# JJanai/slowflow

Hardware: AMD Instinct MI355X
Metric: Mpix*solver-iters/s at 1024x436 (whole coarse-to-fine path) (higher is better)
Workload: dtype f32

## Files before the change

### include/slowflow_amd.h

```cpp
#ifndef SLOWFLOW_AMD_H
#define SLOWFLOW_AMD_H

#include <stddef.h>

#ifdef __cplusplus
extern "C" {
#endif

#define SFA_VERSION 1
#define SFA_MAX_REF 8

typedef enum {
    SFA_OK = 0,
    SFA_ERR_ARG = -1,
    SFA_ERR_HIP = -2,
    SFA_ERR_NO_DEVICE = -3,
    SFA_ERR_REF_FRAME = -4,
    SFA_ERR_TIMEOUT = -5,
    SFA_ERR_UNSUPPORTED = -6
} sfa_status;

typedef struct sfa_image { int width, height, stride; float *data; } sfa_image;
typedef struct sfa_color_image { int width, height, stride; float *c1, *c2, *c3; } sfa_color_image;

// ... 263 lines not shown
int  sfa_job_download_alternation_occlusions(sfa_job *job, int b, int alter, float *occ, int stride);
double sfa_job_mpix_iters(const sfa_job *job);
double sfa_job_device_bytes(const sfa_job *job);

typedef enum { SFA_DEV_F32 = 0, SFA_DEV_U8 = 1, SFA_DEV_U16 = 2 } sfa_dev_dtype;
typedef struct sfa_dev_layout { int dtype; long long window, frame, channel, row, column; } sfa_dev_layout;
void sfa_dev_layout_default(sfa_dev_layout *l, int w, int h, int n_frames);
int  sfa_job_upload_device(sfa_job *job, int b0, int n, const void *frames_dev, const sfa_dev_layout *layout, const float *const chw[3]);
int  sfa_job_set_flow_device(sfa_job *job, int b0, int n, const float *flow_dev, const long long strides[4]);
int  sfa_job_download_device(sfa_job *job, int b0, int n, float *flow_dev, const long long strides[4], float *occ_dev, const long long occ_strides[3]);
int  sfa_job_changes(const sfa_job *job, int b0, int n, float *out);
int  sfa_sequence_upload_device(sfa_sequence *seq, int f0, int n, const void *frames_dev, const sfa_dev_layout *layout);
int  sfa_pair_job_upload_device(sfa_pair_job *job, int b0, int n, const void *frames_dev, const sfa_dev_layout *layout);
int  sfa_pair_job_set_flow_device(sfa_pair_job *job, int b0, int n, const float *flow_dev, const long long strides[4]);
int  sfa_pair_job_download_device(sfa_pair_job *job, int b0, int n, float *flow_dev, const long long strides[4]);
typedef struct sfa_mosaic_desc { int dtype; long long frame, row, column; int W, H, x0, y0; } sfa_mosaic_desc;
int  sfa_demosaic_device(sfa_ctx *ctx, int n, const void *mosaic_dev, const sfa_mosaic_desc *desc, int method, int red_x, int red_y, float *dst_dev,
                         const long long dst_strides[4], int w, int h);
int  sfa_sequence_upload_mosaic_device(sfa_sequence *seq, int f0, int n, const void *mosaic_dev, const sfa_mosaic_desc *desc, int method, int red_x, int red_y);
int  sfa_sequence_upload_mosaic(sfa_sequence *seq, int f, const void *mosaic_host, int dtype, long long host_stride, int W, int H, int x0, int y0, int method,
                                int red_x, int red_y);
int  sfa_job_set_raw_weights(sfa_job *job, int b0, int n, int red_x, int red_y, float weight);
int  sfa_sequence_rescale(sfa_sequence *dst_seq, int f_dst, sfa_sequence *src_seq, int f_src, int n, float scale);

int  sfa_ctx_wait_stream(sfa_ctx *ctx, void *stream);
int  sfa_ctx_signal_stream(sfa_ctx *ctx, void *stream);

typedef struct sfa_sor_batch sfa_sor_batch;
int  sfa_sor_batch_create(sfa_ctx *ctx, int w, int h, int batch, sfa_sor_batch **out);
void sfa_sor_batch_destroy(sfa_sor_batch *sb);
int  sfa_sor_batch_upload(sfa_sor_batch *sb, int b, const float *du, const float *dv, const float *a11, const float *a12,
                          const float *a22, const float *b1, const float *b2, const float *sh, const float *sv, int stride);
int  sfa_sor_batch_run(sfa_sor_batch *sb, int iterations, float omega);
int  sfa_sor_batch_download(sfa_sor_batch *sb, int b, float *du, float *dv, int stride);

int  sfa_ctx_set_wait_bound(sfa_ctx *ctx, unsigned spins);

int  sfa_debug_set(const char *name, const char *value);
int  sfa_ctx_set_verbose(sfa_ctx *ctx, int on);

int  sfa_pair_job_download_system(sfa_pair_job *job, int b, float *a11, float *a12, float *a22, float *b1, float *b2, int stride);

int  sfa_pyramid_down(sfa_ctx *ctx, float *dst, int dw, int dh, int dstride, const float *src, int sw, int sh, int sstride, int nplanes, int nb, float sigma,
                      int info[3]);
int  sfa_resize_flow(sfa_ctx *ctx, float *dwx, float *dwy, int dw, int dh, int dstride, const float *swx, const float *swy, int sw, int sh, int sstride, int nb,
                     float post_x, float post_y);
int  sfa_job_download_level_frame(sfa_job *job, int b, int level, int f, float *frame3, int stride);

int  sfa_division_chain(sfa_ctx *ctx, const float *numerators, const float *denominators, float *q_chain, float *q_exact, unsigned char *admitted, size_t n);

int  sfa_profile_enable(sfa_ctx *ctx, int on);
int  sfa_profile_read(sfa_ctx *ctx, int *n_sor_launches, double *sor_ms_total, double *sor_bytes_total);
int  sfa_profile_read_kernels(sfa_ctx *ctx, int *n_assembly_launches, double *assembly_ms_total, double *assembly_pixel_terms, char *sor_kernel, int sor_kernel_len);
int  sfa_timer_start(sfa_ctx *ctx);
int  sfa_timer_stop(sfa_ctx *ctx, float *ms);

#ifdef __cplusplus
}
#endif
#endif
```

### slowflow_amd/__init__.py

```python
import ctypes as C
import os
import subprocess
import weakref

import numpy as np

_HERE = os.path.dirname(os.path.abspath(__file__))
LIB_PATH = os.environ.get("SFA_LIB") or os.path.join(_HERE, "libslowflow_amd.so")
MAX_REF = 8
MOSAIC_TILE = (64, 16)
MOSAIC_DTYPES = {"float32": 0, "uint8": 1, "uint16": 2}

_f = C.POINTER(C.c_float)


class SlowflowError(RuntimeError):
    pass


def build(verbose=False):
    out = subprocess.run(["make", "-C", os.path.join(_HERE, "csrc"), "-j4"], capture_output=True, text=True)
    if out.returncode != 0:
        raise SlowflowError("building libslowflow_amd.so failed:\n" + out.stdout + out.stderr)
    if verbose:
# ... 122 lines not shown


def track_fill_params(**kw):
    f = TrackFillParams()
    lib().sfa_track_fill_params_default(C.byref(f))
    for k, v in kw.items():
        assert k in ("epic_skip", "min_size", "epic", "workspace_bytes"), k
        setattr(f, k, v)
    return f


def track_job_bytes(params, fill=None):
    L = lib()
    L.sfa_track_job_bytes.argtypes = [C.POINTER(TrackParams), C.POINTER(C.c_size_t)]
    L.sfa_track_job_bytes_fill.argtypes = [C.POINTER(TrackParams), C.POINTER(TrackFillParams), C.POINTER(C.c_size_t)]
    b = C.c_size_t()
    name = "sfa_track_job_bytes" if fill is None else "sfa_track_job_bytes_fill"
    rc = L.sfa_track_job_bytes(C.byref(params), C.byref(b)) if fill is None else L.sfa_track_job_bytes_fill(C.byref(params), C.byref(fill), C.byref(b))
    if rc != 0:
        raise SlowflowError("%s: %s" % (name, L.sfa_last_error(None).decode()))
    return b.value


EXPORTS = [
    "sfa_device_count", "sfa_ctx_create", "sfa_ctx_destroy", "sfa_last_error", "sfa_ctx_sync", "sfa_params_default",
    "sfa_variational", "sfa_variational_2frame", "sfa_variational_2frame_batch", "sfa_epic_nearest_seeds_batch", "sfa_epic_nn_stage_ms", "sfa_ctx_set_epic_search", "sfa_epic_nn_search_info", "sfa_epic_interpolate_batch", "sfa_epic_fit_stage_ms", "sfa_epic_batch", "sfa_epic_saliency_batch", "sfa_epic_batch_stage_ms", "sfa_params_2frame_default", "sfa_pair_job_create", "sfa_pair_job_destroy", "sfa_pair_job_upload", "sfa_pair_job_run", "sfa_pair_job_download", "sfa_pair_job_download_system", "sfa_flow_magnitude_quantile", "sfa_quantile_ranks", "sfa_flow_magnitude_quantiles_device", "sfa_accumulate_consistent", "sfa_accumulate_consistent_scaled", "sfa_jet_source_default", "sfa_jet_flow_resample", "sfa_jet_occlusion_decode", "sfa_hypothesis_energies_scaled", "sfa_accumulate_grid", "sfa_energy_params_default", "sfa_hypothesis_energies", "sfa_hypothesis_energies_ex", "sfa_dt_smoothness_weight", "sfa_fuse_params_default", "sfa_fuse_hypotheses", "sfa_consistent_regions", "sfa_fill_samples", "sfa_fill_matches", "sfa_fill_trajectories", "variational", "sfa_compute_one_level", "sfa_normalize", "sfa_sor_coupled", "sfa_sor_red_black", "sor_coupled",
    "sfa_image_warp", "sfa_derivative_stack", "sfa_convolve", "sfa_dpsis_weight", "sfa_smoothness", "sfa_sub_laplacian",
    "sfa_add_data_and_match", "sfa_occlusion_costs", "sfa_grid_cut", "sfa_grid_cut_batch", "sfa_gaussian_blur", "sfa_resize_linear", "sfa_resize_linear_fx", "sfa_gaussian_presmooth", "sfa_pyramid_sizes",
    "sfa_pyramid_down", "sfa_resize_flow", "sfa_job_download_level_frame",
    "sfa_sequence_create", "sfa_sequence_destroy", "sfa_sequence_upload", "sfa_sequence_download", "sfa_sequence_normalize", "sfa_sequence_frame_sums", "sfa_normalize_statistics", "sfa_sequence_apply_normalization",
    "sfa_job_create", "sfa_job_destroy", "sfa_job_upload", "sfa_job_upload_resident", "sfa_job_reset_flow", "sfa_job_run", "sfa_job_download", "sfa_job_download_occlusions", "sfa_job_keep_alternation_occlusions", "sfa_job_download_alternation_occlusions", "sfa_job_mpix_iters", "sfa_job_device_bytes",
    "sfa_dev_layout_default", "sfa_job_upload_device", "sfa_job_set_flow_device", "sfa_job_download_device", "sfa_job_changes", "sfa_pair_job_upload_device", "sfa_pair_job_set_flow_device", "sfa_pair_job_download_device", "sfa_sequence_upload_device", "sfa_ctx_wait_stream", "sfa_ctx_signal_stream",
    "sfa_demosaic_device", "sfa_sequence_upload_mosaic_device", "sfa_sequence_upload_mosaic", "sfa_job_set_raw_weights", "sfa_sequence_rescale",
    "sfa_sor_batch_create", "sfa_sor_batch_destroy", "sfa_sor_batch_upload", "sfa_sor_batch_run", "sfa_sor_batch_download",
    "sfa_track_params_default", "sfa_track_job_bytes", "sfa_track_job_create", "sfa_track_job_destroy", "sfa_track_job_upload_flows", "sfa_track_job_upload_frames", "sfa_track_job_upload_flows_device", "sfa_track_job_upload_frames_device", "sfa_track_job_run", "sfa_track_job_download_rate", "sfa_track_job_download_fused", "sfa_track_job_download_best", "sfa_ctx_free_bytes", "sfa_track_job_download_device", "sfa_track_job_stage_ms", "sfa_track_job_upload_occlusions_device", "sfa_track_job_download_rate_device", "sfa_track_job_download_best_device",
    "sfa_track_fill_params_default", "sfa_track_job_bytes_fill", "sfa_track_job_create_fill", "sfa_track_job_upload_fill", "sfa_track_job_upload_fill_device", "sfa_track_job_download_fill", "sfa_track_job_fill_ms", "sfa_track_job_fill_info",
    "sfa_division_chain", "sfa_ctx_set_wait_bound", "sfa_debug_set", "sfa_ctx_set_verbose", "sfa_profile_enable", "sfa_profile_read", "sfa_profile_read_kernels", "sfa_timer_start", "sfa_timer_stop",
]

_lib = None


def lib():
    global _lib
    if _lib is None:
        if not os.path.exists(LIB_PATH):
            raise SlowflowError(f"{LIB_PATH} is missing: build it with slowflow_amd.build() / make -C slowflow_amd/csrc "
                                "(there is no CPU fallback)")
        L = C.CDLL(LIB_PATH)
        L.sfa_last_error.restype = C.c_char_p
        L.sfa_last_error.argtypes = [C.c_void_p]
        L.sfa_job_mpix_iters.restype = C.c_double
        L.sfa_job_mpix_iters.argtypes = [C.c_void_p]
        L.sfa_job_device_bytes.restype = C.c_double
        L.sfa_job_device_bytes.argtypes = [C.c_void_p]
        for name in ("sfa_ctx_destroy", "sfa_job_destroy", "sfa_pair_job_destroy", "sfa_track_job_destroy", "sfa_sor_batch_destroy", "sfa_sequence_destroy"):
            if hasattr(L, name):
                getattr(L, name).restype = None
                getattr(L, name).argtypes = [C.c_void_p]
        _lib = L
    return _lib


def fptr(a):
    assert a.dtype == np.float32 and a.flags["C_CONTIGUOUS"], "fp32 C-contiguous planes only"
    return a.ctypes.data_as(_f)


def stride_of(w):
    return ((w + 3) // 4) * 4
# ... 1036 lines not shown

    def apply_normalization(self, avg, std, f0=0, n=None):
        a, s = (C.c_double * 3)(*avg), (C.c_double * 3)(*std)
        self.ctx._ck(lib().sfa_sequence_apply_normalization(self.h_, f0, self.n - f0 if n is None else n, a, s), "sfa_sequence_apply_normalization")

    def close(self):
        if self.h_:
            if self.ctx.h:
                lib().sfa_sequence_destroy(self.h_)
            self.h_ = C.c_void_p()

    def __del__(self):
        try:
            self.close()
        except Exception:
            pass


class SorBatch:

    def __init__(self, ctx, w, h, batch=1):
        self.ctx, self.w, self.h, self.batch = ctx, w, h, batch
        self.h_ = C.c_void_p()
        ctx._ck(lib().sfa_sor_batch_create(ctx.h, w, h, batch, C.byref(self.h_)), "sfa_sor_batch_create")
        ctx._children.add(self)

    def upload(self, b, du, dv, a11, a12, a22, b1, b2, sh, sv):
        stride = du.shape[1]
        self.ctx._ck(lib().sfa_sor_batch_upload(self.h_, b, *[fptr(a) for a in (du, dv, a11, a12, a22, b1, b2, sh, sv)], stride), "sfa_sor_batch_upload")

    def run(self, iterations, omega):
        self.ctx._ck(lib().sfa_sor_batch_run(self.h_, int(iterations), C.c_float(omega)), "sfa_sor_batch_run")

    def download(self, b):
        stride = stride_of(self.w)
        du, dv = np.zeros((self.h, stride), np.float32), np.zeros((self.h, stride), np.float32)
        self.ctx._ck(lib().sfa_sor_batch_download(self.h_, b, fptr(du), fptr(dv), stride), "sfa_sor_batch_download")
        return du, dv

    def close(self):
        if self.h_:
            if self.ctx.h:
                lib().sfa_sor_batch_destroy(self.h_)
            self.h_ = C.c_void_p()

    def __del__(self):
        try:
            self.close()
        except Exception:
            pass
```

### slowflow_amd/csrc/api.hip

```cpp
#include <algorithm>
#include <cmath>
#include <cstring>
#include <memory>
#include <mutex>

#include "sfa_internal.h"

#pragma clang fp contract(off)

namespace sfa {

thread_local std::string g_thread_err;

#ifndef SFA_RELEASE
Switches g_switches;
static const char *const kSwitchNames[Switches::N] = {
    "SFA_SOR_CHAIN", "SFA_SOR_BAND", "SFA_SOR_F", "SFA_SOR_CH", "SFA_SOR_LEAD", "SFA_CHAIN_LDS", "SFA_RB_TILE", "SFA_WARP_ALLJ", "SFA_NO_WARP_SMOOTH",
    "SFA_ASSEMBLE_GENERIC", "SFA_EXACT_DIV", "SFA_ASM_XCD", "SFA_NO_DIRECT_OPERANDS", "SFA_NO_UV_ALIAS", "SFA_DEBUG_ACTIVE", "SFA_UNFUSED", "SFA_SHARE_SOR",
    "SFA_PYRAMID_UNFUSED", "SFA_CUT_DISCHARGE", "SFA_CUT_INNER", "SFA_CUT_SUPER", "SFA_CUT_TAIL_INNER", "SFA_CUT_PER", "SFA_CUT_TAIL_PER", "SFA_CUT_TAIL_SUPER",
    "SFA_CUT_DEBUG", "SFA_CUT_NO_TAIL", "SFA_CUT_TAIL", "SFA_NO_EXACT_BREAK", "SFA_PAIR_UNFUSED", "SFA_EPIC_FIT_PLAIN", "SFA_EPIC_NN_SET", "SFA_EPIC_NN_SLICE"};
static int set_switch(const char *name, const char *value) {
    for (int i = 0; i < Switches::N; i++)
        if (!strcmp(name, kSwitchNames[i])) {
            g_switches.given[i] = value != nullptr;
            g_switches.value[i] = value ? atoi(value) : 0;
            if (i == Switches::EPIC_NN_SET && value) g_switches.value[i] = !strcmp(value, "sparse") ? 1 : !strcmp(value, "dense") ? 0 : -1;
            return SFA_OK;
        }
    return SFA_ERR_ARG;
}
static void switches_from_environment() {
    static std::once_flag once;
    std::call_once(once, [] {
        const char *d = getenv("SFA_DEBUG");
        if (!d || atoi(d) == 0) return;
        for (int i = 0; i < Switches::N; i++)
            if (const char *e = getenv(kSwitchNames[i])) (void)set_switch(kSwitchNames[i], e);
    });
}
#else
static void switches_from_environment() {}
#endif

int set_error(sfa_ctx *ctx, int code, const char *fmt, ...) {
    char buf[1024];
    va_list ap;
    va_start(ap, fmt);
    vsnprintf(buf, sizeof buf, fmt, ap);
    va_end(ap);
    g_thread_err = buf;
    if (ctx) ctx->err = buf;
    return code;
}
// ... 527 lines not shown
    long pl = 0, es = 0;
    DevMem mem;
    SorWorkspace ws;
    float *plane(int b, int i) const { return mem.f() + b * es + (long)i * pl; }
};

int sfa_sor_batch_create(sfa_ctx *ctx, int w, int h, int batch, sfa_sor_batch **out) {
    CHECK_ARGS(ctx && out && w > 0 && h > 0 && batch > 0 && batch <= kMaxBatch, "bad arguments");
    SFA_HIP(ctx, hipSetDevice(ctx->device));
    std::unique_ptr<sfa_sor_batch> sb(new sfa_sor_batch());
    sb->ctx = ctx; sb->w = w; sb->h = h; sb->nb = batch; sb->pitch = dev_pitch(w);
    sb->pl = (long)sb->pitch * h; sb->es = 9 * sb->pl;
    SFA_TRY(sb->mem.alloc(ctx, (size_t)batch * sb->es * sizeof(float)));
    SFA_HIP(ctx, hipMemsetAsync(sb->mem.p, 0, (size_t)batch * sb->es * sizeof(float), ctx->stream));
    *out = sb.release();
    return SFA_OK;
}
void sfa_sor_batch_destroy(sfa_sor_batch *sb) {
    if (!sb) return;
    (void)hipSetDevice(sb->ctx->device);
    (void)hipStreamSynchronize(sb->ctx->stream);
    delete sb;
}
int sfa_sor_batch_upload(sfa_sor_batch *sb, int b, const float *du, const float *dv, const float *a11, const float *a12, const float *a22, const float *b1,
                         const float *b2, const float *sh, const float *sv, int stride) {
    sfa_ctx *ctx = sb ? sb->ctx : nullptr;
    CHECK_ARGS(sb && b >= 0 && b < sb->nb && du && dv && a11 && a12 && a22 && b1 && b2 && sh && sv && stride >= sb->w, "bad arguments");
    SFA_HIP(ctx, hipSetDevice(ctx->device));
    const float *src[9] = {du, dv, a11, a12, a22, b1, b2, sh, sv};
    for (int i = 0; i < 9; i++) SFA_TRY(upload_plane(ctx, sb->plane(b, i), sb->pitch, src[i], stride, sb->w, sb->h));
    SFA_HIP(ctx, hipStreamSynchronize(ctx->stream));
    return SFA_OK;
}
int sfa_sor_batch_run(sfa_sor_batch *sb, int iterations, float omega) {
    sfa_ctx *ctx = sb ? sb->ctx : nullptr;
    CHECK_ARGS(sb, "null batch");
    SFA_HIP(ctx, hipSetDevice(ctx->device));
    Geo g{sb->w, sb->h, sb->pitch, sb->pl, sb->es, sb->nb, WMask::first(sb->nb), nullptr};
    return sor_run(ctx, sb->ws, g, sb->plane(0, 0), sb->plane(0, 1), sb->plane(0, 2), sb->plane(0, 3), sb->plane(0, 4), sb->plane(0, 5), sb->plane(0, 6),
                   sb->plane(0, 7), sb->plane(0, 8), iterations, omega, true);
}
int sfa_sor_batch_download(sfa_sor_batch *sb, int b, float *du, float *dv, int stride) {
    sfa_ctx *ctx = sb ? sb->ctx : nullptr;
    CHECK_ARGS(sb && b >= 0 && b < sb->nb && du && dv && stride >= sb->w, "bad arguments");
    SFA_HIP(ctx, hipSetDevice(ctx->device));
    SFA_TRY(download_plane(ctx, du, stride, sb->plane(b, 0), sb->pitch, sb->w, sb->h));
    SFA_TRY(download_plane(ctx, dv, stride, sb->plane(b, 1), sb->pitch, sb->w, sb->h));
    return sfa_ctx_sync(ctx);
}

int sfa_sor_coupled(sfa_ctx *ctx, sfa_image *du, sfa_image *dv, sfa_image *a11, sfa_image *a12, sfa_image *a22, sfa_image *b1, sfa_image *b2,
                    sfa_image *dpsis_horiz, sfa_image *dpsis_vert, int iterations, float omega) {
    CHECK_ARGS(ctx && du && dv && a11 && a12 && a22 && b1 && b2 && dpsis_horiz && dpsis_vert, "null image");
    const int w = du->width, h = du->height, stride = du->stride;
    CHECK_ARGS(w > 0 && h > 0 && stride >= w, "bad image geometry");
    sfa_image *im[9] = {du, dv, a11, a12, a22, b1, b2, dpsis_horiz, dpsis_vert};
    for (auto *i : im) CHECK_ARGS(i->data && i->width == w && i->height == h && i->stride == stride, "images must share one geometry");
    Staging s;
    SFA_TRY(s.init(ctx, w, h, 9));
    for (int i = 0; i < 9; i++) SFA_TRY(s.up(i, im[i]->data, stride));
    SorWorkspace ws;
    SFA_TRY(sor_run(ctx, ws, s.geo(), s.plane(0), s.plane(1), s.plane(2), s.plane(3), s.plane(4), s.plane(5), s.plane(6), s.plane(7), s.plane(8), iterations,
                    omega, true));
    SFA_TRY(s.down(du->data, stride, 0)); SFA_TRY(s.down(dv->data, stride, 1));
    if (!(w < 2 || h < 2 || iterations < 1))
        for (int i = 2; i < 5; i++) SFA_TRY(s.down(im[i]->data, stride, i));
// ... 378 lines not shown
```

### slowflow_amd/csrc/job.hip

```cpp
#include <algorithm>
#include <cmath>
#include <cstring>
#include <memory>
#include <vector>

#include "sfa_internal.h"

#pragma clang fp contract(off)

namespace sfa {

enum { P_WX = 0, P_WY, P_UU, P_VV, P_DU, P_DV, P_ODU, P_ODV, P_SH, P_SV, P_A11, P_A12, P_A22, P_B1, P_B2, P_OCC, P_DPSIS, P_COUNT };
struct Level {
    int w = 0, h = 0, pitch = 0, lstride = 0, ref = 0, F = 0, nb = 0;
    bool fused = true;
    long pl = 0, es = 0;
    long off_masks = 0, off_warp = 0, off_stacks = 0, off_tmp = 0;
    float *base = nullptr;
    float *pbase = nullptr;
    float *plane(int i) const { return i < 2 ? pbase + (long)i * pl : base + (long)(i - 2) * pl; }
    float *mask(int s) const { return base + off_masks + (long)s * pl; }
    float *stack(int s, int toref) const { return base + off_stacks + ((long)s * 2 + toref) * 24 * pl; }
    float *warp(int s, int sp1) const { return base + off_warp + (long)(s + sp1) * 3 * pl; }
    float *frame(int f) const { return pbase + 2 * pl + (long)f * 3 * pl; }
// ... 189 lines not shown
    SFA_HIP(c, hipStreamSynchronize(c->stream));
    for (int b = 0; b < L.nb; b++)
        if (close.test(b) && std::max(hx[2 * b], hx[2 * b + 1]) < p.thres_inner) in_active.clear(b);
    return SFA_OK;
}

static int inner_iterations(sfa_ctx *c, const Level &L, const sfa_params &p, const LevelPlan &P, AssembleArgs &aa, SorWorkspace &sorws, const Geo &g, bool smoothed) {
    if (!P.direct) launch_zero_planes(c, g, P.du, 2);
    WMask in_active = g.active, outer_done = WMask::none();
    for (int inner = 0; inner < p.niter_inner; inner++) {
        Geo gi = g;
        gi.active = in_active;
        const bool first_zero = P.direct && inner == 0;
        SFA_TRY(assemble_and_solve(c, L, p, P, aa, sorws, gi, first_zero, smoothed && inner == 0));
        if (update_flow(c, p, P, aa.op, gi, inner, first_zero)) outer_done = in_active;
        if (P.verbose) print_changes(c, L, "\tinner it", inner, in_active);
        if (P.thres_in && inner + 1 < p.niter_inner) {
            SFA_TRY(inner_break(c, L, p, P, gi, in_active));
            if (!in_active.any()) break;
        }
    }
    if (outer_done != g.active) {
        Geo go = g;
        go.active = g.active.andnot(outer_done);
        launch_update_outer(c, go, P.wx, P.wy, P.uu, P.vv, c->d_red, P.dfa, P.dfb);
    }
    return SFA_OK;
}
static int run_level(sfa_ctx *c, const Level &L, const sfa_params &p, const ChannelWeights &cw, SorWorkspace &sorws, DevMem &cut_scratch, float *change, float *occ_log) {
    AssembleArgs aa;
    bool need_toref[2 * SFA_MAX_REF] = {false};
    SFA_TRY(data_terms(c, L, p, cw, aa, need_toref));
    const LevelPlan P(c, L, p);
    const OuterBreak brk{c, P.thres_out};
    const WMask all = WMask::first(L.nb);
    Geo g = L.geo(all);
    launch_fill_planes(c, g, P.occ, 1, (p.one_direction || p.occlusion_reasoning) ? -1.0f : 0.0f);
    launch_dpsis(c, g, P.dpsis, L.frame(L.ref), L.es, 5.0f, p.norm_avg, p.norm_std, p.hbit);
    if (!P.uv_alias) launch_copy_planes(c, g, P.uu, P.wx, 2, L.es, L.es);
    g.amask = c->d_amask;
    SFA_HIP(c, hipMemsetAsync(c->d_last, 0, sizeof(LastBlock), c->stream));
    launch_set_mask(c, all);

    for (int alter = 0; alter < p.niter_alter; alter++) {
        WMask active = all;
        g.active = active;
        if (P.thres_out && alter > 0) launch_set_mask(c, all);
        bool smoothed = get_derivatives(c, L, p, g, need_toref, P.uv_alias);
        if (alter > 0 && p.occlusion_reasoning && !p.one_direction) SFA_TRY(optimize_occlusions(c, L, p, g, cut_scratch));
        if (alter > 0 && p.occlusion_reasoning && occ_log)
            launch_copy_planes(c, g, occ_log + (long)alter * L.pl, P.occ, 1, (long)p.niter_alter * L.pl, L.es);
        for (int outer = 0; outer < p.niter_outer; outer++) {
            SFA_TRY(brk.known(outer, active));
            if (!active.any()) break;
            if (sw_given(Switches::DEBUG_ACTIVE)) fprintf(stderr, "level %dx%d alter %d outer %d known active %d\n", L.w, L.h, alter, outer, active.count());
            g.active = active;
            if (outer > 0) smoothed = get_derivatives(c, L, p, g, need_toref, P.uv_alias);
            if (!L.fused) launch_mask_weight(c, g, L.mask(0), P.occ, aa.data_norm, L.ref, p.one_direction);
            SFA_TRY(inner_iterations(c, L, p, P, aa, sorws, g, smoothed));
            if (P.verbose) print_changes(c, L, "outer it", outer, active);
            const bool last_iter = (alter == p.niter_alter - 1 && outer == p.niter_outer - 1);
            if (P.thres_out || last_iter) launch_outer_threshold(c, g, c->d_red, P.thres_out ? p.thres_outer : 0.0f, P.dfa, P.dfb);
            SFA_TRY(brk.publish(outer));
        }
    }
    if (change) {
// ... 422 lines not shown
```

### slowflow_amd/csrc/kernels.hip

```cpp
#include "sfa_device.h"
#include "sor_device.h"

#pragma clang fp contract(off)

namespace sfa {

__device__ __forceinline__ float psi_vec(const PenaltyDev &p, float xsq) {
    const float e2 = p.eps * p.eps;
    switch (p.id) {
    case 0: return 1.0f;
    case 2: return __fdiv_rn(1.0f, 2.0f * e2 + xsq);
    case 3: {
        float out = __fdiv_rn(1.0f, 2.0f * sqrt_rn(xsq + e2));
        if (sqrt_rn(xsq) > p.trunc) out = 0.0f;
        return out;
    }
    case 4: {
        float t = e2 + xsq;
        t = t * t;
        return __fdiv_rn(e2 + 2.0f * xsq, t);
    }
    default: return __fdiv_rn(1.0f, 2.0f * sqrt_rn(xsq + e2));
    }
}
// ... 1304 lines not shown
            p.ixz[ch] = d5x_in(sZ[ch], cz);
        }
    }
    return p;
}
template <class K>
__device__ __forceinline__ void asm_epilogue_pixel(const AssembleArgs &a, const Geo &g, Acc &A, float u, float v, int x0, int y0, int tx, int yl, int x, int y) {
    const float *const lds = asm_lds<K>();
    const int gy0 = y0 + DT_H - 1;
    const TileAcc U{lds, x0, gy0}, V{lds + K::GR * DT_W, x0, gy0}, Hh{lds + 2 * K::GR * DT_W, x0, gy0}, Wv{lds + 3 * K::GR * DT_W, x0, gy0};
    if (a.do_laplacian) {
        A.b1 = laplacian_gather(A.b1, U, Hh, Wv, x, y, g.w, g.h);
        A.b2 = laplacian_gather(A.b2, V, Hh, Wv, x, y, g.w, g.h);
    }
    if (!a.op.sa) return;
    const float hp = Hh(x, y);
    const float hl = x > 0 ? Hh(x - 1, y) : 0.0f;
    const float vp = Wv(x, y);
    const float vt = y > 0 ? Wv(x, y - 1) : 0.0f;
    const PointBlock q = sor_point_block(hl, hp, vt, vp, y, g.h, A.a11, A.a12, A.a22);
    const OperandTile<K> T;
    T.A[yl][tx] = make_float4(q.i11, q.i12, q.i22, vt);
    T.B[yl][tx] = make_float4(A.b1, A.b2, hp, y < g.h - 1 ? vp : 0.0f);
    T.X[yl][tx] = make_float2(u, v);
}
template <class K>
__device__ __forceinline__ void asm_store_operand_tile(const SorOperandOut &op, const Geo &g, int b, int c0, int r0) {
    const OperandTile<K> T;
    for (int item = threadIdx.x; item < (DT_X + K::TY - 1) * K::TY; item += K::NT) {
        const int dl = item / K::TY, rl = item % K::TY, cl = dl - rl;
        if (cl < 0 || cl >= DT_X) continue;
        const int r = r0 + rl, c = c0 + cl;
        if (r >= g.h || c >= g.w) continue;
        const size_t e = diag_entry(b, op.ent, op.RP, op.G, c, r);
        if (SFA_X_AI & 64) continue;
        const float2 xv = T.X[rl][cl];
        op.sa[e] = T.A[rl][cl];
        op.sb[e] = T.B[rl][cl];
        op.x[e] = f2u(xv.x, xv.y);
    }
}

template <int TY, int NT, int MINB, bool ZUV, int FAST, bool XT>
__global__ void __launch_bounds__(NT, MINB) k_assemble_images(AssembleArgs a, const float *__restrict__ base, float *__restrict__ a11, float *__restrict__ a12,
                                                              float *__restrict__ a22, float *__restrict__ b1, float *__restrict__ b2,
                                                              const float *__restrict__ du, const float *__restrict__ dv, const float *__restrict__ uu,
                                                              const float *__restrict__ vv, const float *__restrict__ sh, const float *__restrict__ sv,
                                                              const float *__restrict__ occ, Geo g, XcdTiles xt) {
    using K = AsmTile<TY, NT>;
    constexpr int NR = K::NR, NP = K::NP;
    float *const lds = asm_lds<K>();
#ifdef SFA_ASM_TIMING
    unsigned long long at_acc[14] = {0}, at_t = __builtin_readcyclecounter();
#endif
    int bx, by, b;
    if (!asm_block_tile<XT>(g, xt, bx, by, b)) return;
    asm_reset_progress<K>(a.op, bx, by, b);
    if (!elem_active(g, b)) return;
    const int x0 = bx * DT_X - DT_H, y0 = by * TY - DT_H;
    const bool tile_in = SFA_TILE_FAST && x0 >= 0 && x0 + DT_W <= g.w && y0 >= 0 && y0 + K::TR <= g.h;
    const long eb = b * g.es;
    const int tx = threadIdx.x & 63;
    const int ty = __builtin_amdgcn_readfirstlane(threadIdx.x >> 6);
    const int x = x0 + DT_H + tx;
    const int dt_norm = FAST ? 1 : a.dt_norm;
    PenaltyDev pcolor = a.color, pgrad = a.grad;
    if (FAST) { pcolor.id = FAST; pgrad.id = FAST; }
// ... 165 lines not shown
    const int wid = threadIdx.y, lane = threadIdx.x;
    if (lane == 0) { sm[wid] = a; sm[BY + wid] = b; }
    __syncthreads();
    if (wid == 0 && lane == 0) {
        double sa = 0, sb = 0;
        for (int i = 0; i < BY; i++) { sa += sm[i]; sb += sm[BY + i]; }
        a = sa; b = sb;
    }
}

__global__ void __launch_bounds__(BX *BY) k_update_inner(float *__restrict__ uu, float *__restrict__ vv, const float *__restrict__ wx, const float *__restrict__ wy,
                                                          const float *__restrict__ du, const float *__restrict__ dv, const float *__restrict__ odu,
                                                          const float *__restrict__ odv, double *__restrict__ partial, float *__restrict__ dfa, float *__restrict__ dfb, Geo g) {
    const int b = blockIdx.z;
    const int x = blockIdx.x * BX + threadIdx.x;
    double sa = 0, sb = 0;
    if (elem_active(g, b) && x < g.w)
        for (int y = blockIdx.y * BY + threadIdx.y; y < g.h; y += gridDim.y * BY) {
            const size_t o = b * g.es + (size_t)y * g.pitch + x;
            const float d = du[o], e = dv[o];
            sa += (double)fabsf(odu[o] - d);
            sb += (double)fabsf(odv[o] - e);
            if (dfa) { dfa[o] = fabsf(odu[o] - d); dfb[o] = fabsf(odv[o] - e); }
            uu[o] = wx[o] + d;
            vv[o] = wy[o] + e;
        }
    block_sum2(sa, sb);
    if (threadIdx.x == 0 && threadIdx.y == 0) {
        const size_t blk = ((size_t)b * gridDim.y + blockIdx.y) * gridDim.x + blockIdx.x;
        partial[2 * blk] = sa; partial[2 * blk + 1] = sb;
    }
}
__global__ void __launch_bounds__(BX *BY) k_update_inner_x(float *__restrict__ uu, float *__restrict__ vv, const float *__restrict__ wx, const float *__restrict__ wy,
                                                            const unsigned long long *__restrict__ xs, long ent, int RP, int G, const float *__restrict__ odu,
                                                            const float *__restrict__ odv, float *__restrict__ du_out, float *__restrict__ dv_out,
                                                            double *__restrict__ partial, float *__restrict__ dfa, float *__restrict__ dfb, Geo g) {
    const int b = blockIdx.z;
    const int x = blockIdx.x * BX + threadIdx.x;
    double sa = 0, sb = 0;
    if (elem_active(g, b) && x < g.w)
        for (int y = blockIdx.y * BY + threadIdx.y; y < g.h; y += gridDim.y * BY) {
            const size_t o = b * g.es + (size_t)y * g.pitch + x;
            const unsigned long long xv = xs[diag_entry(b, ent, RP, G, x, y)];
            const float d = __uint_as_float((unsigned)(xv & 0xffffffffu)), e = __uint_as_float((unsigned)(xv >> 32));
            const float od = odu ? odu[o] : 0.0f, oe = odv ? odv[o] : 0.0f;
            sa += (double)fabsf(od - d);
            sb += (double)fabsf(oe - e);
            if (dfa) { dfa[o] = fabsf(od - d); dfb[o] = fabsf(oe - e); }
            uu[o] = wx[o] + d;
            vv[o] = wy[o] + e;
            if (du_out) { du_out[o] = d; dv_out[o] = e; }
        }
    block_sum2(sa, sb);
    if (threadIdx.x == 0 && threadIdx.y == 0) {
        const size_t blk = ((size_t)b * gridDim.y + blockIdx.y) * gridDim.x + blockIdx.x;
        partial[2 * blk] = sa; partial[2 * blk + 1] = sb;
    }
}
template <bool FUSE>
__global__ void __launch_bounds__(BX *BY) k_update_outer_x(float *__restrict__ uu, float *__restrict__ vv, float *__restrict__ wx, float *__restrict__ wy,
                                                            const unsigned long long *__restrict__ xs, long ent, int RP, int G, double *__restrict__ partial,
                                                            double *__restrict__ out, unsigned *__restrict__ done, float *__restrict__ dfa, float *__restrict__ dfb, Geo g) {
    __shared__ unsigned long long tX[16][67];
    const int b = blockIdx.z;
    const int tid = threadIdx.y * BX + threadIdx.x;
    const int c0 = blockIdx.x * 64;
    double sa = 0, sb = 0;
    if (!elem_active(g, b)) return;
    {
        for (int r0 = blockIdx.y * 16; r0 < g.h; r0 += gridDim.y * 16) {
            __syncthreads();
            for (int item = tid; item < (64 + 16 - 1) * 16; item += BX * BY) {
                const int dl = item / 16, rl = item % 16, cl = dl - rl;
                if (cl < 0 || cl >= 64) continue;
                const int r = r0 + rl, c = c0 + cl;
                if (r < g.h && c < g.w) tX[rl][cl] = xs[diag_entry(b, ent, RP, G, c, r)];
            }
            __syncthreads();
            const int x = c0 + threadIdx.x;
            if (x < g.w)
#pragma unroll
                for (int k = 0; k < 4; k++) {
                    const int rl = threadIdx.y + 4 * k, y = r0 + rl;
                    if (y >= g.h) break;
                    const size_t o = b * g.es + (size_t)y * g.pitch + x;
                    const unsigned long long xv = tX[rl][threadIdx.x];
                    const float d = __uint_as_float((unsigned)(xv & 0xffffffffu)), e = __uint_as_float((unsigned)(xv >> 32));
                    const float ox = wx[o], oy = wy[o];
                    const float u = ox + d, v = oy + e;
                    sa += (double)fabsf(u - ox);
                    sb += (double)fabsf(v - oy);
                    if (uu) { uu[o] = u; vv[o] = v; }
                    if (dfa) { dfa[o] = fabsf(u - ox); dfb[o] = fabsf(v - oy); }
#if defined(SFA_UPD_NT) && SFA_UPD_NT
                    __builtin_nontemporal_store(u, wx + o); __builtin_nontemporal_store(v, wy + o);
#else
                    wx[o] = u; wy[o] = v;
#endif
                }
        }
    }
    block_sum2(sa, sb);
    if (!FUSE) {
        if (tid == 0) {
            const size_t blk = ((size_t)b * gridDim.y + blockIdx.y) * gridDim.x + blockIdx.x;
            partial[2 * blk] = sa; partial[2 * blk + 1] = sb;
        }
        return;
    }
// ... 123 lines not shown
    if (!which.test(b)) return;
    float fa, fd;
    exact_norms(dfa + b * g.es, dfb + b * g.es, g, lane, fa, fd);
    if (lane == 0) { out[2 * b] = fa; out[2 * b + 1] = fd; }
}
void launch_exact_norms(sfa_ctx *c, const Geo &g, const float *dfa, const float *dfb, const WMask &which, float *out) {
    hipLaunchKernelGGL(k_exact_norms, dim3(g.nb), dim3(64), 0, c->stream, dfa, dfb, out, which, g);
}
__global__ void k_set_mask(unsigned long long *amask, WMask v) { for (int i = 0; i < kMaskWords; i++) amask[i] = v.w[i]; }
static unsigned long long *unsure_of(sfa_ctx *c) { return c->d_last->unsure; }
void launch_outer_threshold(sfa_ctx *c, const Geo &g, const double *red, float thres, const float *dfa, const float *dfb) {
    const bool exact = dfa && thres > 0.0f;
    hipLaunchKernelGGL(k_outer_threshold, dim3(kMaskWords), dim3(64), 0, c->stream, red, c->d_last->last, c->d_amask, g.active, g.nb, (double)g.h * g.w, thres,
                       exact ? unsure_of(c) : (unsigned long long *)nullptr, break_band(g.w, g.h));
    if (exact) hipLaunchKernelGGL(k_exact_break, dim3(g.nb), dim3(64), 0, c->stream, dfa, dfb, c->d_last->last, c->d_amask, unsure_of(c), g, thres);
}
void launch_set_mask(sfa_ctx *c, const WMask &v) { hipLaunchKernelGGL(k_set_mask, dim3(1), dim3(1), 0, c->stream, c->d_amask, v); }

static double *partials_of(sfa_ctx *c) { return c->d_red + 2 * kMaxBatch; }
constexpr int kRedRows = 16;
static inline dim3 red_grid(const Geo &g, int z) { return dim3((g.w + BX - 1) / BX, std::min((g.h + BY - 1) / BY, kRedRows), z); }

void launch_update_inner(sfa_ctx *c, const Geo &g, float *uu, float *vv, const float *wx, const float *wy, const float *du, const float *dv,
                         const float *old_du, const float *old_dv, double *red, float *dfa, float *dfb) {
    dim3 grid = red_grid(g, g.nb);
    const int per_elem = grid.x * grid.y;
    hipLaunchKernelGGL(k_update_inner, grid, block2d(), 0, c->stream, uu, vv, wx, wy, du, dv, old_du, old_dv, partials_of(c), dfa, dfb, g);
    hipLaunchKernelGGL(k_reduce_partials, dim3(g.nb), dim3(256), 0, c->stream, partials_of(c), per_elem, red, g.active, g.amask);
}
void launch_update_inner_x(sfa_ctx *c, const Geo &g, float *uu, float *vv, const float *wx, const float *wy, const SorOperandOut &x, const float *old_du,
                           const float *old_dv, float *du_out, float *dv_out, double *red, float *dfa, float *dfb) {
    dim3 grid = red_grid(g, g.nb);
    const int per_elem = grid.x * grid.y;
    hipLaunchKernelGGL(k_update_inner_x, grid, block2d(), 0, c->stream, uu, vv, wx, wy, x.x, x.ent, x.RP, x.G, old_du, old_dv, du_out, dv_out, partials_of(c), dfa, dfb, g);
    hipLaunchKernelGGL(k_reduce_partials, dim3(g.nb), dim3(256), 0, c->stream, partials_of(c), per_elem, red, g.active, g.amask);
}
constexpr int kFuseReduceWindows = 4;
void launch_update_outer_x(sfa_ctx *c, const Geo &g, float *uu, float *vv, float *wx, float *wy, const SorOperandOut &x, double *red, float *dfa, float *dfb) {
    dim3 grid((g.w + 63) / 64, std::min((g.h + 15) / 16, kRedRows), g.nb);
    const int per_elem = grid.x * grid.y;
    unsigned *done = c->d_last->done;
    if (g.nb <= kFuseReduceWindows) {
        hipLaunchKernelGGL(k_update_outer_x<true>, grid, block2d(), 0, c->stream, uu, vv, wx, wy, x.x, x.ent, x.RP, x.G, partials_of(c), red, done, dfa, dfb, g);
        return;
    }
    hipLaunchKernelGGL(k_update_outer_x<false>, grid, block2d(), 0, c->stream, uu, vv, wx, wy, x.x, x.ent, x.RP, x.G, partials_of(c), red, done, dfa, dfb, g);
    hipLaunchKernelGGL(k_reduce_partials, dim3(g.nb), dim3(256), 0, c->stream, partials_of(c), per_elem, red, g.active, g.amask);
}
void launch_update_outer(sfa_ctx *c, const Geo &g, float *wx, float *wy, const float *uu, const float *vv, double *red, float *dfa, float *dfb) {
    dim3 grid = red_grid(g, g.nb);
    const int per_elem = grid.x * grid.y;
    hipLaunchKernelGGL(k_update_outer, grid, block2d(), 0, c->stream, wx, wy, uu, vv, partials_of(c), dfa, dfb, g);
    hipLaunchKernelGGL(k_reduce_partials, dim3(g.nb), dim3(256), 0, c->stream, partials_of(c), per_elem, red, g.active, g.amask);
}

__global__ void k_copy_planes(float *__restrict__ dst, const float *__restrict__ src, Geo g, int nplanes, long dst_es, long src_es) {
    const int b = blockIdx.z / nplanes, pl = blockIdx.z % nplanes;
    if (!elem_active(g, b)) return;
    const int x = blockIdx.x * BX + threadIdx.x, y = blockIdx.y * BY + threadIdx.y;
    if (x >= g.w || y >= g.h) return;
    const size_t o = pl * g.pl + (size_t)y * g.pitch + x;
    dst[b * dst_es + o] = src[b * src_es + o];
}
void launch_copy_planes(sfa_ctx *c, const Geo &g, float *dst, const float *src, int nplanes, long dst_es, long src_es) {
    hipLaunchKernelGGL(k_copy_planes, grid2d(g, nplanes), block2d(), 0, c->stream, dst, src, g, nplanes, dst_es, src_es);
}

__global__ void k_fill_planes(float *__restrict__ p, Geo g, int nplanes, float v) {
    const int b = blockIdx.z / nplanes, pl = blockIdx.z % nplanes;
    if (!elem_active(g, b)) return;
    const int x = blockIdx.x * BX + threadIdx.x, y = blockIdx.y * BY + threadIdx.y;
    if (x >= g.pitch || y >= g.h) return;
    p[b * g.es + pl * g.pl + (size_t)y * g.pitch + x] = v;
}
void launch_fill_planes(sfa_ctx *c, const Geo &g, float *p, int nplanes, float v) {
    dim3 grid((g.pitch + BX - 1) / BX, (g.h + BY - 1) / BY, g.nb * nplanes);
    hipLaunchKernelGGL(k_fill_planes, grid, block2d(), 0, c->stream, p, g, nplanes, v);
}
void launch_zero_planes(sfa_ctx *c, const Geo &g, float *p, int nplanes) { launch_fill_planes(c, g, p, nplanes, 0.0f); }
// ... 436 lines not shown
```

### slowflow_amd/csrc/sfa_internal.h

```cpp
#pragma once
#include <hip/hip_runtime.h>

#include <cstdarg>
#include <cstdio>
#include <string>
#include <vector>

#include "../../include/slowflow_amd.h"
#include "dev_view.h"

#pragma clang fp contract(off)

namespace sfa {

constexpr int kMaskWords = 2;
constexpr int kMaxBatch = 64 * kMaskWords;
struct WMask {
    unsigned long long w[kMaskWords];
    __host__ __device__ bool test(int b) const { return (w[b >> 6] >> (b & 63)) & 1ull; }
    __host__ __device__ void clear(int b) { w[b >> 6] &= ~(1ull << (b & 63)); }
    __host__ __device__ void set(int b) { w[b >> 6] |= 1ull << (b & 63); }
    __host__ __device__ bool any() const { unsigned long long o = 0; for (int i = 0; i < kMaskWords; i++) o |= w[i]; return o != 0; }
    __host__ __device__ bool operator==(const WMask &o) const { bool e = true; for (int i = 0; i < kMaskWords; i++) e = e && w[i] == o.w[i]; return e; }
    __host__ __device__ bool operator!=(const WMask &o) const { return !(*this == o); }
// ... 43 lines not shown
    size_t ev_used = 0;
    double sor_bytes = 0;
    std::vector<hipEvent_t> ev2;
    size_t ev2_used = 0;
    double asm_pixel_terms = 0;
    char sor_kernel[160] = {0};
    void *rb_tmp = nullptr;
    size_t rb_tmp_bytes = 0;
    void *q_tmp = nullptr;
    size_t q_tmp_bytes = 0;
    float epic_ms[5] = {};
    int epic_search = 0;
    long long epic_info[4] = {};
    float epic_fit_ms[2] = {};
    float epic_batch_ms[8] = {};
    int epic_chain_runs[2] = {};
    hipEvent_t t0 = nullptr, t1 = nullptr;
    hipEvent_t ev_wait = nullptr, ev_signal = nullptr;
    bool verbose_changes = false;
    int cu_count = 256;
};

namespace sfa {

constexpr int kRedDoubles = 1 << 20;

int set_error(sfa_ctx *ctx, int code, const char *fmt, ...);
extern thread_local std::string g_thread_err;

struct Switches {
    enum Id {
        SOR_CHAIN, SOR_BAND, SOR_F, SOR_CH, SOR_LEAD, CHAIN_LDS, RB_TILE, WARP_ALLJ, NO_WARP_SMOOTH, ASSEMBLE_GENERIC, EXACT_DIV, ASM_XCD, NO_DIRECT_OPERANDS,
        NO_UV_ALIAS, DEBUG_ACTIVE, UNFUSED, SHARE_SOR, PYRAMID_UNFUSED, CUT_DISCHARGE, CUT_INNER, CUT_SUPER, CUT_TAIL_INNER, CUT_PER, CUT_TAIL_PER, CUT_TAIL_SUPER,
        CUT_DEBUG, CUT_NO_TAIL, CUT_TAIL, NO_EXACT_BREAK, PAIR_UNFUSED, EPIC_FIT_PLAIN, EPIC_NN_SET, EPIC_NN_SLICE, N
    };
    bool given[N] = {};
    int value[N] = {};
};
#ifdef SFA_RELEASE
#define SFA_FULL(...)
#else
#define SFA_FULL(...) __VA_ARGS__
#endif
#ifdef SFA_RELEASE
constexpr bool sw_given(Switches::Id) { return false; }
constexpr int sw_int(Switches::Id, int dflt) { return dflt; }
#else
extern Switches g_switches;
inline bool sw_given(Switches::Id i) { return g_switches.given[i]; }
inline int sw_int(Switches::Id i, int dflt) { return g_switches.given[i] ? g_switches.value[i] : dflt; }
#endif

#define SFA_HIP(ctx, call)                                                                         \
    do {                                                                                           \
        hipError_t _e = (call);                                                                    \
        if (_e != hipSuccess)                                                                      \
            return sfa::set_error((ctx), SFA_ERR_HIP, "%s failed: %s (%s:%d)", #call, hipGetErrorString(_e), __FILE__, __LINE__); \
    } while (0)

#define SFA_TRY(expr)            \
    do {                         \
        int _rc = (expr);        \
        if (_rc != SFA_OK) return _rc; \
    } while (0)

#define CHECK_ARGS_FN(fn, cond, msg) do { if (!(cond)) return sfa::set_error(ctx, SFA_ERR_ARG, "%s: %s", fn, msg); } while (0)
#define CHECK_ARGS(cond, msg) CHECK_ARGS_FN(__func__, cond, msg)
// ... 93 lines not shown
struct EpicChainDev { const float *const *cost; const float *const *matches; const int *nm; const float *const *sal; float *const *fx; float *const *fy; };
int epic_chain_device(sfa_ctx *ctx, const char *fn, int n, int w, int h, const sfa_epic_params *p, const EpicChainDev &io, int *rc, int (*counts)[3],
                      size_t workspace_bytes, int *status);

struct Geo { int w, h, pitch; long pl; long es; int nb; WMask active; const unsigned long long *amask; };

struct PenaltyDev { int id; float eps, trunc; };
inline PenaltyDev pen(const sfa_penalty &p) { return PenaltyDev{p.id, p.eps, p.trunc}; }

struct WarpJob { long src_off, dst_off, mask_off; int factor; };
struct WarpJobs { WarpJob job[4 * SFA_MAX_REF]; int n; };
void launch_warp_jobs(sfa_ctx *c, const Geo &g, const WarpJobs &J, float *base, const float *wx, const float *wy);
bool launch_warp_smooth(sfa_ctx *c, const Geo &g, const WarpJobs &J, float *base, const float *wx, const float *wy, int method, float *sh, float *sv,
                        const float *dpsis, float alpha, PenaltyDev reg);
void launch_warp(sfa_ctx *c, const Geo &g, float *dst3, float *mask, const float *src3, const float *wx, const float *wy, int factor,
                 long src_es );
void launch_deriv_stack(sfa_ctx *c, const Geo &g, float *out24, const float *I1, const float *I2, long es1, long es2);
void launch_convolve(sfa_ctx *c, const Geo &g, float *dst, const float *src, int order, int horiz, int nplanes);
void launch_dpsis(sfa_ctx *c, const Geo &g, float *dst, const float *im3, long im_es, float coef, const float avg[3], const float stdv[3], int hbit);
void launch_smoothness(sfa_ctx *c, const Geo &g, int method, float *sh, float *sv, const float *uu, const float *vv, const float *dpsis,
                       float alpha, PenaltyDev reg);
void launch_sub_laplacian(sfa_ctx *c, const Geo &g, float *dst, const float *src, const float *wh, const float *wv);
void launch_mask_weight(sfa_ctx *c, const Geo &g, float *masks, const float *occ, float data_norm, int ref, int one_direction);
void launch_fill(sfa_ctx *c, float *p, size_t n, float v);
void launch_division_chain(sfa_ctx *c, const float *a, const float *b, float *q_chain, float *q_exact, unsigned char *admitted, size_t n);
void launch_fill_planes(sfa_ctx *c, const Geo &g, float *p, int nplanes, float v);
void launch_zero_planes(sfa_ctx *c, const Geo &g, float *p, int nplanes);
void launch_outer_threshold(sfa_ctx *c, const Geo &g, const double *red, float thres, const float *dfa = nullptr, const float *dfb = nullptr);
void launch_set_mask(sfa_ctx *c, const WMask &v);

struct SorOperandOut {
    float4 *sa = nullptr, *sb = nullptr; unsigned long long *x = nullptr; unsigned *flags = nullptr;
    long ent = 0; int RP = 0, G = 0, ntasks = 0, nb = 0;
};
struct Term {
    long stack_off; long mask_off; float hd, hg, s; int is_ref;
    long i1_off, i2_off; int backward;
};
struct AssembleArgs {
    Term t[kMaxTerms];
    int n;
    int dt_norm;
    PenaltyDev color, grad;
    const float *chw; long chw_pl; long chw_es; int chw_pitch; int chw_stride0; int lstride;
    int accumulate;
    int do_laplacian;
    float data_norm; int one_direction;
    SorOperandOut op;
    int zero_duv;
    int chain_ok = 0;
};
void launch_assemble(sfa_ctx *c, const Geo &g, const AssembleArgs &a, const float *base , float *a11, float *a12,
                     float *a22, float *b1, float *b2, const float *du, const float *dv, const float *uu, const float *vv, const float *sh, const float *sv);

int launch_assemble_images(sfa_ctx *c, const Geo &g, const AssembleArgs &a, const float *base, float *a11, float *a12, float *a22, float *b1, float *b2,
                            const float *du, const float *dv, const float *uu, const float *vv, const float *sh, const float *sv, const float *occ);

void launch_smoothness_2f(sfa_ctx *c, const Geo &g, float *sh, float *sv, const float *uu, const float *vv, const float *dpsis, float half_alpha);
void launch_data_2f(sfa_ctx *c, const Geo &g, const float *D, const float *mask, const float *du, const float *dv, float *a11, float *a12, float *a22, float *b1,
                    float *b2, const float *wx, const float *wy, const float *sh, const float *sv, float hd, float hg);
void launch_data_2f_fused(sfa_ctx *c, const Geo &g, const float *I1, const float *I2, const float *mask, const float *du, const float *dv, float *a11, float *a12,
                          float *a22, float *b1, float *b2, const float *wx, const float *wy, const float *sh, const float *sv, float hd, float hg);

struct OccSlot {
    long s1_off, s2_off;
    long r1_off, r2_off;
// ... 25 lines not shown
                        long ses, int nb, float post_x, float post_y);
void launch_resize_scaled(sfa_ctx *c, float *dst, int dw, int dh, int dpitch, long dpl, long des, const float *src, int sw, int sh, int spitch, long spl,
                          long ses, int nplanes, int nb, float post_scale, double scale_x, double scale_y);
struct PyrInfo { int fused, td, lds; };
bool launch_pyr_down(sfa_ctx *c, float *dst, int dw, int dh, int dpitch, long dpl, long des, const float *src, int sw, int sh, int spitch, long spl, long ses,
                     int nplanes, int nb, const float *taps, int radius, PyrInfo *info = nullptr);
int pyramid_step(sfa_ctx *c, float *dst, int dw, int dh, int dpitch, long dpl, long des, const float *src, int sw, int sh, int spitch, long spl, long ses, int nplanes,
                 int nb, const float *taps, int radius, float *tmp, PyrInfo *info = nullptr);
void launch_presmooth(sfa_ctx *c, const Geo &g, float *dst, float *tmp, const float *src, int nplanes, float sigma);
void launch_normalize_sums(sfa_ctx *c, const Geo &g, const float *frames3, double *red );
void launch_normalize_apply(sfa_ctx *c, const Geo &g, float *frames3, const double avg[3], const double stdv[3]);
__attribute__((visibility("hidden"))) int cv_gauss_taps(float sigma, float k[kMaxBlurTaps]);

struct PackSrc { const void *p; int dtype; long long sw, sf, sc, sr, sx; };
void launch_pack_frames(sfa_ctx *c, float *dst, long dst_es, long pl, int pitch, int w, int h, int nwin, int F, const PackSrc &s);
void launch_pack_flow(sfa_ctx *c, float *dst, long dst_es, long pl, int pitch, int w, int h, int nwin, const float *src, const long long st[4]);
void launch_unpack_planes(sfa_ctx *c, const float *wx, const float *wy, const float *occ, long src_es, int pitch, int w, int h, int nwin, float *flow,
                          const long long st[4], float *occ_dst, const long long ost[3]);

struct MosaicSrc { const void *p; int dtype; long long sf, sr, sx; int W, H, x0, y0; };
struct MosaicDst { float *p; long long sf, sc, sr, sx; int w, h; };
void launch_demosaic(sfa_ctx *c, const MosaicSrc &src, const MosaicDst &dst, int n, int method, int red_x, int red_y);
void launch_raw_weights(sfa_ctx *c, float *chw, long es, long pl, int cp, int stride, int w, int h, int nwin, int red_x, int red_y, float weight);

struct SorWorkspace {
    sfa_ctx *ctx = nullptr;
    int w = 0, h = 0, K = 0, nb = 0;
    int NB = 0, NG = 0, RP = 0, ND = 0, G = 0, NS = 0, NCH = 0, ntasks = 0, F = 0, CHK = 0;
    int nwords = 0;
    long ent = 0;
    int band = 0, Wp = 0, EP = 0;
    int chain = 0;
    long edge_job = 0;
    DevMem sa, sb, x, flags, order, edge;
    int configure(sfa_ctx *ctx, int w, int h, int K, int nb);
};
int sor_operand_target(sfa_ctx *c, SorWorkspace &ws, const Geo &g, int K, SorOperandOut *out);
int sor_run_prepared(sfa_ctx *c, SorWorkspace &ws, const Geo &g, float *du, float *dv, int K, float omega);
int sor_rb_run(sfa_ctx *c, const Geo &g, float *du, float *dv, float *a11, float *a12, float *a22, const float *b1, const float *b2, const float *sh,
               const float *sv, int K, float omega);
int sor_run(sfa_ctx *c, SorWorkspace &ws, const Geo &g, float *du, float *dv, float *a11, float *a12, float *a22, const float *b1, const float *b2,
            const float *sh, const float *sv, int K, float omega, bool inv_out);

__attribute__((visibility("hidden"))) int check_view(sfa_ctx *ctx, const char *fn, const View &v, long long min_inner = 1);
__attribute__((visibility("hidden"))) int check_disjoint(sfa_ctx *ctx, const char *fn, std::initializer_list<View> views, const char *why = nullptr);
int check_frames_source(sfa_ctx *ctx, const char *fn, const void *frames_dev, const sfa_dev_layout *l, long long win_stride, int nwin, int F, int w, int h);
int check_device_pointer(sfa_ctx *ctx, const char *fn, const char *arg, const void *p, long long last, size_t elem);
int check_download_destination(sfa_ctx *ctx, const char *fn, int n, int w, int h, float *flow_dev, const long long strides[4], float *occ_dev,
                               const long long occ_strides[3]);
int check_batch_range(sfa_ctx *ctx, const char *fn, const char *what, int b0, int n, int nb);
__attribute__((visibility("hidden"))) int check_mosaic_method(sfa_ctx *ctx, const char *fn, int method, int red_x, int red_y);

}

struct sfa_pair_job {
    enum { WX, WY, UU, VV, DU, DV, SH, SV, A11, A12, A22, B1, B2, MASK, DPS, IM1, IM2 = IM1 + 3, WIM2 = IM2 + 3, NPL = WIM2 + 3 };
    sfa_ctx *ctx = nullptr;
    int w = 0, h = 0, n = 0, pitch = 0;
    long pl = 0, es = 0;
    sfa_params_2frame p;
    bool stored_stack = false;
    sfa::DevMem mem;
    sfa::DevMem stack;
    sfa::SorWorkspace ws;
    float *plane(int b, int i) const { return mem.f() + b * es + (long)i * pl; }
    sfa::Geo geo() const { return sfa::Geo{w, h, pitch, pl, es, n, sfa::WMask::first(n), nullptr}; }
// ... 17 lines not shown
```

### slowflow_amd/csrc/sor.hip

```cpp
#include <type_traits>

#include "sfa_internal.h"
#include "sfa_device.h"
#include "sor_device.h"

#pragma clang fp contract(off)

namespace sfa {

#ifndef SFA_BAND_STARTLAG
#define SFA_BAND_STARTLAG 2
#endif
#ifndef SFA_PUBLISH_VMCNT
#define SFA_PUBLISH_VMCNT (2 * CH - 1)
#endif

#ifndef SFA_PROGRESS_STRIDE
#define SFA_PROGRESS_STRIDE 32
#endif
constexpr int kProgressStride = SFA_PROGRESS_STRIDE;

struct SorArgs {
    const float4 *sa;
    const float4 *sb;
// ... 494 lines not shown
    constexpr int WINA = 2 * (FA - 1) * (64 + FA - 1) * 32, WINB_ = FB > 1 ? 2 * (FB - 1) * (64 + FB - 1) * 32 : 0;
    unsigned char *win0 = smem + (size_t)(NW - 1) * RING * 64 * 8 + 256;
    unsigned long long(*est0)[MC] = reinterpret_cast<unsigned long long(*)[MC]>(win0 + (size_t)NA * WINA + (size_t)NB_ * WINB_);
    constexpr int TVB = (FA + 1) * CH;
    unsigned long long *tvb0 = reinterpret_cast<unsigned long long *>(est0 + (size_t)NW * FA);
    unsigned &s_ticket = lprog[NW];
    const int lane = threadIdx.x & 63;
    const int wave = __builtin_amdgcn_readfirstlane(threadIdx.x >> 6);
    if (threadIdx.x == 0) s_ticket = atomicAdd(a.gflags + (size_t)a.nb * a.NB * NW * kProgressStride, 1u);
    if (threadIdx.x < NW) lprog[threadIdx.x] = 0;
    __syncthreads();
    const unsigned t = __builtin_amdgcn_readfirstlane(s_ticket);
    if (t >= (unsigned)(a.nb * a.NB)) return;
    const int job = t % a.nb, b = t / a.nb;
    if (!elem_active(a.active, a.amask, job)) return;
    unsigned char *win = wave < NA ? win0 + (size_t)wave * WINA : win0 + (size_t)NA * WINA + (size_t)(wave - NA) * WINB_;
    unsigned long long(*est)[MC] = est0 + (size_t)wave * FA;
    unsigned long long *tvb = tvb0 + (size_t)wave * TVB;
    const int k0 = wave < NA ? wave * FA : NA * FA + (wave - NA) * FB;
    if (wave == 0)                   band_wave<FA, CH, MC, RING, 0, FA>(a, ring, lprog, win, est, tvb, job, b, wave, lane, k0);
    else if (wave < NA)              band_wave<FA, CH, MC, RING, 1, FA>(a, ring, lprog, win, est, tvb, job, b, wave, lane, k0);
    else if (wave == NA && NB_ == 1) band_wave<FB, CH, MC, RING, 2, FA>(a, ring, lprog, win, est, tvb, job, b, wave, lane, k0);
    else if (wave == NA)             band_wave<FB, CH, MC, RING, 1, FA>(a, ring, lprog, win, est, tvb, job, b, wave, lane, k0);
    else if (wave == NW - 1)         band_wave<FB, CH, MC, RING, 2, FB>(a, ring, lprog, win, est, tvb, job, b, wave, lane, k0);
    else                             band_wave<FB, CH, MC, RING, 1, FB>(a, ring, lprog, win, est, tvb, job, b, wave, lane, k0);
}

struct PrepArgs {
    float4 *sa; float4 *sb; unsigned long long *x; unsigned *flags;
    const float *du, *dv, *b1, *b2, *sh, *sv;
    float *a11, *a12, *a22;
    long ent, es;
    int W, H, RP, ND, G, pitch, ntasks, nb, inv_out;
    WMask active; const unsigned long long *amask;
};
constexpr int PT_C = 64, PT_R = 16;
__global__ void __launch_bounds__(256) k_sor_prepare(PrepArgs p) {
    __shared__ float4 tA[PT_R][PT_C + 2];
    __shared__ float4 tB[PT_R][PT_C + 2];
    __shared__ float2 tX[PT_R][PT_C + 3];
    const int job = blockIdx.z;
    const int c0 = blockIdx.x * PT_C, r0 = blockIdx.y * PT_R;
    const int tx = threadIdx.x & 63, ty = threadIdx.x >> 6;
    if (blockIdx.x == 0 && blockIdx.y == 0) {
        for (int i = threadIdx.x; i < p.ntasks; i += 256) p.flags[(size_t)job * p.ntasks + i] = 0;
        if (job == 0 && threadIdx.x == 0) p.flags[(size_t)p.nb * p.ntasks] = 0;
    }
    if (!elem_active(p.active, p.amask, job)) return;
#pragma unroll
    for (int i = 0; i < PT_R / 4; i++) {
        const int rl = ty + 4 * i, r = r0 + rl, c = c0 + tx;
        if (r < p.H && c < p.W) {
            const size_t o = (size_t)job * p.es + (size_t)r * p.pitch + c;
            const float hp = p.sh[o];
            const float hl = c > 0 ? p.sh[o - 1] : 0.0f;
            const float vp = p.sv[o];
            const float vt = r > 0 ? p.sv[o - p.pitch] : 0.0f;
            const PointBlock q = sor_point_block(hl, hp, vt, vp, r, p.H, p.a11[o], p.a12[o], p.a22[o]);
            tA[rl][tx] = make_float4(q.i11, q.i12, q.i22, vt);
            tB[rl][tx] = make_float4(p.b1[o], p.b2[o], hp, r < p.H - 1 ? vp : 0.0f);
            tX[rl][tx] = make_float2(p.du[o], p.dv[o]);
            if (p.inv_out) { p.a11[o] = q.i11; p.a12[o] = q.i12; p.a22[o] = q.i22; }
        }
    }
    __syncthreads();
    for (int item = threadIdx.x; item < (PT_C + PT_R - 1) * PT_R; item += 256) {
        const int dl = item / PT_R, rl = item % PT_R, cl = dl - rl;
        if (cl < 0 || cl >= PT_C) continue;
        const int r = r0 + rl, c = c0 + cl;
        if (r >= p.H || c >= p.W) continue;
        const size_t e = diag_entry(job, p.ent, p.RP, p.G, c, r);
        p.sa[e] = tA[rl][cl];
        p.sb[e] = tB[rl][cl];
        const float2 xv = tX[rl][cl];
        p.x[e] = f2u(xv.x, xv.y);
    }
}

__global__ void k_sor_finish(float *__restrict__ du, float *__restrict__ dv, const unsigned long long *__restrict__ x, long ent, long es, int W, int H,
                             int RP, int G, int pitch, WMask active, const unsigned long long *__restrict__ amask) {
    const int job = blockIdx.z;
    const int c = blockIdx.x * 64 + threadIdx.x, r = blockIdx.y * 4 + threadIdx.y;
    if (c >= W || r >= H || !elem_active(active, amask, job)) return;
    const float2 v = u2f(x[diag_entry(job, ent, RP, G, c, r)]);
    const size_t o = (size_t)job * es + (size_t)r * pitch + c;
    du[o] = v.x;
    dv[o] = v.y;
}

__global__ void k_sor_readable(float *du_, float *dv_, const float *a11_, const float *a12_, const float *a22_, const float *b1_, const float *b2_,
                               const float *sh_, const float *sv_, long es, int w, int h, int stride, int iterations, float omega,
                               WMask active, const unsigned long long *amask) {
    if (threadIdx.x != 0 || !elem_active(active, amask, blockIdx.x)) return;
    const long eb = (long)blockIdx.x * es;
    float *du = du_ + eb, *dv = dv_ + eb;
    const float *a11 = a11_ + eb, *a12 = a12_ + eb, *a22 = a22_ + eb, *b1 = b1_ + eb, *b2 = b2_ + eb, *sh = sh_ + eb, *sv = sv_ + eb;
    for (int iter = 0; iter < iterations; iter++)
        for (int j = 0; j < h; j++)
            for (int i = 0; i < w; i++) {
                const size_t o = (size_t)j * stride + i;
                float sigma_u = 0.0f, sigma_v = 0.0f, sum_dpsis = 0.0f;
                if (j > 0) { sigma_u -= sv[o - stride] * du[o - stride]; sigma_v -= sv[o - stride] * dv[o - stride]; sum_dpsis += sv[o - stride]; }
                if (i > 0) { sigma_u -= sh[o - 1] * du[o - 1]; sigma_v -= sh[o - 1] * dv[o - 1]; sum_dpsis += sh[o - 1]; }
                if (j < h - 1) { sigma_u -= sv[o] * du[o + stride]; sigma_v -= sv[o] * dv[o + stride]; sum_dpsis += sv[o]; }
                if (i < w - 1) { sigma_u -= sh[o] * du[o + 1]; sigma_v -= sh[o] * dv[o + 1]; sum_dpsis += sh[o]; }
                const float A11 = a11[o] + sum_dpsis, A12 = a12[o], A22 = a22[o] + sum_dpsis;
                const float det = A11 * A22 - A12 * A12;
                const float B1 = b1[o] - sigma_u, B2 = b2[o] - sigma_v;
                du[o] = (1.0f - omega) * du[o] + __fdiv_rn(omega * (A22 * B1 - A12 * B2), det);
                dv[o] = (1.0f - omega) * dv[o] + __fdiv_rn(omega * (-A12 * B1 + A11 * B2), det);
            }
}

__global__ void __launch_bounds__(256) k_rb_invert(float *__restrict__ a11, float *__restrict__ a12, float *__restrict__ a22, const float *__restrict__ sh,
                                                   const float *__restrict__ sv, Geo g) {
    const int b = blockIdx.z;
    if (!elem_active(g, b)) return;
// ... 124 lines not shown
        float *tu = static_cast<float *>(c->rb_tmp), *tv = tu + (size_t)g.nb * pl;
        const dim3 grid((g.w + 63) / 64, (g.h + 15) / 16, g.nb);
        bool in_tmp = false;
        for (int k = 0; k < K; k += T) {
            const int ns = std::min(T, K - k);
            const float *iu = in_tmp ? tu : du, *iv = in_tmp ? tv : dv;
            float *ou = in_tmp ? du : tu, *ov = in_tmp ? dv : tv;
            const long ei = in_tmp ? pl : g.es, eo = in_tmp ? g.es : pl;
#ifndef SFA_RELEASE
            if (T == 3) hipLaunchKernelGGL((k_rb_tile<3>), grid, dim3(256), 0, c->stream, iu, iv, ei, g.pitch, ou, ov, eo, g.pitch, a11, a12, a22, b1, b2, sh, sv, g, ns, omega);
            else
#endif
                        hipLaunchKernelGGL((k_rb_tile<5>), grid, dim3(256), 0, c->stream, iu, iv, ei, g.pitch, ou, ov, eo, g.pitch, a11, a12, a22, b1, b2, sh, sv, g, ns, omega);
            in_tmp = !in_tmp;
        }
        if (in_tmp) {
            Geo gc = g;
            launch_copy_planes(c, gc, du, tu, 1, g.es, pl);
            launch_copy_planes(c, gc, dv, tv, 1, g.es, pl);
        }
    }
    if (prof) {
        (void)hipEventRecord(c->ev[c->ev_used + 1], c->stream);
        c->ev_used += 2;
        c->sor_bytes += (44.0 * K + 12.0) * (double)g.w * g.h * g.nb;
    }
    SFA_HIP(c, hipGetLastError());
    return SFA_OK;
}

bool chain_shape(int id, int K, int *KG, int *NW, int *FMAX);
int chain_ch();
int chain_shift(int id);
void chain_kernel_name(int id, int NG, char *buf, size_t n);
int chain_flag_stride();
int chain_ah();
int sor_chain_launch(sfa_ctx *c, SorWorkspace &ws, const Geo &g, int K, float omega);

static int chain_choice(int K, int nb, int NBands) {
    int id = 0;
    if (sw_given(Switches::SOR_CHAIN)) id = sw_int(Switches::SOR_CHAIN, 0);
    else if (sw_given(Switches::SOR_BAND) || sw_given(Switches::SOR_F)) id = 0;
    else {
        const int bands = nb * NBands;
        static const int lone[] = {16, 6, 1, 2, 5, 3, 0}, few[] = {6, 1, 2, 5, 3, 0}, many[] = {14, 11, 3, 5, 2, 6, 1, 0};
        int KG, NW, FMAX;
        for (const int *cand = bands <= 32 ? lone : bands <= 72 ? few : many; *cand; cand++)
            if (chain_shape(*cand, K, &KG, &NW, &FMAX)) { id = *cand; break; }
    }
    int KG, NW, FMAX;
    if (id > 0 && !chain_shape(id, K, &KG, &NW, &FMAX)) id = 0;
    return id;
}
static int band_shape(int K, int nb) {
#ifdef SFA_RELEASE
    (void)K; (void)nb;
    return 0;
#endif
    int F = nb >= 8 ? 43 : 0;
    F = sw_int(Switches::SOR_BAND, F);
    if (F == 43) { if (K == 30) return 43; F = 5; }
    if (F <= 0 || F > 6 || F == 4) return 0;
    auto fits = [&](int f) { return f >= 1 && K % f == 0 && K / f <= (f == 6 ? 5 : f == 5 ? 6 : f == 3 ? 10 : 16); };
    if (fits(F)) return F;
    if (fits(5)) return 5;
    if (fits(3)) return 3;
// ... 2 lines not shown
    return 0;
}
#ifndef SFA_BAND_CH3
#define SFA_BAND_CH3 4
#endif
#ifndef SFA_BAND_CH2
#define SFA_BAND_CH2 2
#endif
#ifndef SFA_BAND_CH5
#define SFA_BAND_CH5 4
#endif
constexpr int band_ch(int F) { return F == 3 ? SFA_BAND_CH3 : F == 5 ? SFA_BAND_CH5 : F == 6 ? 5 : F == 2 ? SFA_BAND_CH2 : 2; }
#ifndef SFA_BAND_MC3
#define SFA_BAND_MC3 12
#endif
#ifndef SFA_BAND_MC2
#define SFA_BAND_MC2 8
#endif
#ifndef SFA_BAND_MC5
#define SFA_BAND_MC5 8
#endif
constexpr int band_mc(int F) { return F == 3 ? SFA_BAND_MC3 : F == 2 ? SFA_BAND_MC2 : F == 5 ? SFA_BAND_MC5 : F == 6 ? 10 : 8; }
static int band_ring(int F) { return F == 2 ? 8 : 16; }
static size_t band_window(int F) { return F > 1 ? (size_t)2 * (F - 1) * (64 + F - 1) * 32 : 0; }

static void sor_shape(int K, int nwaves1, int &F, int &CHK) {
    F = nwaves1 >= 900 ? 2 : 1; CHK = F == 1 ? 16 : 8;
    F = sw_int(Switches::SOR_F, F);
    CHK = sw_int(Switches::SOR_CH, CHK);
    if (!((F == 1 && (CHK == 8 || CHK == 16)) || (F == 2 && (CHK == 8 || CHK == 4)) || (F == 3 && CHK == 4))) { F = 2; CHK = 8; }
    if (K % F != 0) { F = 1; CHK = 16; }
}

int SorWorkspace::configure(sfa_ctx *c, int w_, int h_, int K_, int nb_) {
    int F_, CH_;
    const int chain_ = chain_choice(K_, nb_, (h_ + K_ - 1 + 63) / 64);
    const int band_ = chain_ ? 0 : band_shape(K_, nb_);
    if (chain_) { F_ = 0; CH_ = chain_ch(); }
    else if (band_ == 43) { F_ = 4; CH_ = 12; }
    else if (band_) { F_ = band_; CH_ = band_mc(band_); }
    else sor_shape(K_, nb_ * ((h_ + K_ - 1 + 63) / 64) * K_, F_, CH_);
    if (ctx == c && w == w_ && h == h_ && K == K_ && nb == nb_ && F == F_ && CHK == CH_ && band == band_ && chain == chain_) return SFA_OK;
    ctx = c; w = w_; h = h_; K = K_; nb = nb_; F = F_; CHK = CH_; band = band_; chain = chain_;
    NB = (h + K - 1 + 63) / 64;
    if (chain) {
        int KG, NW, FMAX;
        chain_shape(chain, K, &KG, &NW, &FMAX);
        const int CH = chain_ch(), AH = chain_ah(), LEAD = AH + 1;
        NG = K / KG;
#ifndef SFA_GUARD_ALIGN
#define SFA_GUARD_ALIGN 8
#endif
        G = round_up(K + 64, SFA_GUARD_ALIGN);
        RP = round_up(h + 2 * G, 16);
        NCH = round_up((w + 64 + KG - NW + 2 * CH + FMAX + CH - 1) / CH + chain_shift(chain), 4);
        NS = round_up(NCH + LEAD + NW + 2, AH);
        ND = NS * CH + 64 * NB + G + 32;
        ntasks = NB * NG;
        nwords = ntasks * chain_flag_stride();
        ent = (long)ND * RP;
        EP = 256;
        Wp = round_up(EP + NS * CH + 64 + 2 * K + 64, 8);
        edge_job = (long)NB * K * Wp;
        SFA_TRY(edge.alloc(c, (size_t)nb * edge_job * sizeof(unsigned long long)));
        SFA_HIP(c, hipMemsetAsync(edge.p, 0, (size_t)nb * edge_job * sizeof(unsigned long long), c->stream));
        SFA_TRY(sa.alloc(c, (size_t)nb * ent * sizeof(float4)));
        SFA_TRY(sb.alloc(c, (size_t)nb * ent * sizeof(float4)));
        SFA_TRY(x.alloc(c, (size_t)nb * ent * sizeof(unsigned long long)));
        SFA_TRY(flags.alloc(c, ((size_t)nb * nwords + 16) * sizeof(unsigned)));
        SFA_TRY(order.alloc(c, (size_t)NB * NG * sizeof(int2)));
        SFA_HIP(c, hipMemsetAsync(sa.p, 0, (size_t)nb * ent * sizeof(float4), c->stream));
        SFA_HIP(c, hipMemsetAsync(sb.p, 0, (size_t)nb * ent * sizeof(float4), c->stream));
        SFA_HIP(c, hipMemsetAsync(x.p, 0, (size_t)nb * ent * sizeof(unsigned long long), c->stream));
        std::vector<int2> ord;
        ord.reserve(NB * NG);
        for (int key = 0; key <= 3 * (NB - 1) + (NG - 1); key++)
            for (int b = 0; b < NB; b++) {
                const int g = key - 3 * b;
                if (g >= 0 && g < NG) ord.push_back(make_int2(b, g));
            }
        SFA_HIP(c, hipMemcpyAsync(order.p, ord.data(), ord.size() * sizeof(int2), hipMemcpyHostToDevice, c->stream));
        SFA_HIP(c, hipStreamSynchronize(c->stream));
        return SFA_OK;
    }
    NG = band == 43 ? 8 : (K + F - 1) / F;
    G = K + 64;
    RP = round_up(h + 2 * G, 16);
    NS = w + 63 + F - 1;
    NCH = (NS + CHK - 1) / CHK;
    if (band) NS = NCH * CHK;
    ND = w + 64 * NB + 2 * CHK + F + 2 * G + 8;
    ntasks = NB * NG;
    nwords = ntasks * kProgressStride;
    ent = (long)ND * RP;
    if (band) {
        EP = 72;
        Wp = round_up(EP + NS + 2 * CHK + 8, 8);
        edge_job = (long)NB * K * Wp;
        SFA_TRY(edge.alloc(c, (size_t)nb * edge_job * sizeof(unsigned long long)));
        SFA_HIP(c, hipMemsetAsync(edge.p, 0, (size_t)nb * edge_job * sizeof(unsigned long long), c->stream));
    }
    SFA_TRY(sa.alloc(c, (size_t)nb * ent * sizeof(float4)));
    SFA_TRY(sb.alloc(c, (size_t)nb * ent * sizeof(float4)));
    SFA_TRY(x.alloc(c, (size_t)nb * ent * sizeof(unsigned long long)));
    SFA_TRY(flags.alloc(c, ((size_t)nb * nwords + 16) * sizeof(unsigned)));
    SFA_TRY(order.alloc(c, (size_t)ntasks * sizeof(int2)));
    SFA_HIP(c, hipMemsetAsync(sa.p, 0, (size_t)nb * ent * sizeof(float4), c->stream));
    SFA_HIP(c, hipMemsetAsync(sb.p, 0, (size_t)nb * ent * sizeof(float4), c->stream));
    SFA_HIP(c, hipMemsetAsync(x.p, 0, (size_t)nb * ent * sizeof(unsigned long long), c->stream));
    std::vector<int2> ord;
    ord.reserve(ntasks);
    for (int key = 0; key <= 3 * (NB - 1) + (NG - 1); key++)
        for (int b = 0; b < NB; b++) {
            const int g = key - 3 * b;
            if (g >= 0 && g < NG) ord.push_back(make_int2(b, g));
        }
    SFA_HIP(c, hipMemcpyAsync(order.p, ord.data(), ord.size() * sizeof(int2), hipMemcpyHostToDevice, c->stream));
    SFA_HIP(c, hipStreamSynchronize(c->stream));
    return SFA_OK;
}

int sor_operand_target(sfa_ctx *c, SorWorkspace &ws, const Geo &g, int K, SorOperandOut *out) {
    if (g.w < 2 || g.h < 2 || K < 1) return set_error(c, SFA_ERR_ARG, "sor_operand_target: system too small for the pipelined solver");
    SFA_TRY(ws.configure(c, g.w, g.h, K, g.nb));
    out->sa = (float4 *)ws.sa.p; out->sb = (float4 *)ws.sb.p; out->x = (unsigned long long *)ws.x.p; out->flags = (unsigned *)ws.flags.p;
    out->ent = ws.ent; out->RP = ws.RP; out->G = ws.G; out->ntasks = ws.nwords; out->nb = g.nb;
    return SFA_OK;
}

static int sor_launch_solve(sfa_ctx *c, SorWorkspace &ws, const Geo &g, float *du, float *dv, int K, float omega);

int sor_run(sfa_ctx *c, SorWorkspace &ws, const Geo &g, float *du, float *dv, float *a11, float *a12, float *a22, const float *b1, const float *b2,
            const float *sh, const float *sv, int K, float omega, bool inv_out) {
    if (g.w < 2 || g.h < 2 || K < 1) {
        hipLaunchKernelGGL(k_sor_readable, dim3(g.nb), dim3(64), 0, c->stream, du, dv, a11, a12, a22, b1, b2, sh, sv, g.es, g.w, g.h, g.pitch, K, omega,
                           g.active, g.amask);
        return SFA_OK;
    }
    SFA_TRY(ws.configure(c, g.w, g.h, K, g.nb));
    PrepArgs p;
    p.sa = (float4 *)ws.sa.p; p.sb = (float4 *)ws.sb.p; p.x = (unsigned long long *)ws.x.p; p.flags = (unsigned *)ws.flags.p;
    p.du = du; p.dv = dv; p.b1 = b1; p.b2 = b2; p.sh = sh; p.sv = sv; p.a11 = a11; p.a12 = a12; p.a22 = a22;
    p.ent = ws.ent; p.es = g.es; p.W = g.w; p.H = g.h; p.RP = ws.RP; p.ND = ws.ND; p.G = ws.G; p.pitch = g.pitch;
    p.ntasks = ws.nwords; p.nb = g.nb; p.inv_out = inv_out ? 1 : 0; p.active = g.active; p.amask = g.amask;
    hipLaunchKernelGGL(k_sor_prepare, dim3((g.w + PT_C - 1) / PT_C, (g.h + PT_R - 1) / PT_R, g.nb), dim3(256), 0, c->stream, p);
    return sor_launch_solve(c, ws, g, du, dv, K, omega);
}

int sor_run_prepared(sfa_ctx *c, SorWorkspace &ws, const Geo &g, float *du, float *dv, int K, float omega) {
    if (ws.ctx != c || ws.w != g.w || ws.h != g.h || ws.K != K || ws.nb != g.nb) return set_error(c, SFA_ERR_ARG, "sor_run_prepared: workspace not configured for this system");
    return sor_launch_solve(c, ws, g, du, dv, K, omega);
}

static int sor_launch_solve(sfa_ctx *c, SorWorkspace &ws, const Geo &g, float *du, float *dv, int K, float omega) {
    struct { float4 *sa, *sb; unsigned long long *x; unsigned *flags; } p{(float4 *)ws.sa.p, (float4 *)ws.sb.p, (unsigned long long *)ws.x.p, (unsigned *)ws.flags.p};
    SorArgs a;
    a.sa = p.sa; a.sb = p.sb; a.x = p.x; a.flags = p.flags; a.order = (const int2 *)ws.order.p; a.err = c->d_err;
    a.ent = ws.ent; a.W = g.w; a.H = g.h; a.K = K; a.NB = ws.NB; a.NG = ws.NG; a.RP = ws.RP; a.G = ws.G; a.NS = ws.NS; a.NCH = ws.NCH;
    a.ntasks = ws.ntasks; a.nwords = ws.nwords; a.nb = g.nb; a.omega = omega; a.active = g.active; a.amask = g.amask;
    const bool prof = c->profile && c->ev_used + 2 <= c->ev.size();
    if (prof) (void)hipEventRecord(c->ev[c->ev_used], c->stream);
    if (ws.chain) chain_kernel_name(ws.chain, ws.NG, c->sor_kernel, sizeof c->sor_kernel);
    else if (ws.band == 43) snprintf(c->sor_kernel, sizeof c->sor_kernel, "k_sor_band_mixed<4,6,3,2,4,12,16>");
    else if (ws.band) snprintf(c->sor_kernel, sizeof c->sor_kernel, "k_sor_band<%d>", ws.F);
    else snprintf(c->sor_kernel, sizeof c->sor_kernel, "k_sor_solve<%d,%d>", ws.F, ws.CHK);
    if (ws.chain) {
        SFA_TRY(sor_chain_launch(c, ws, g, K, omega));
    }
#ifndef SFA_RELEASE
    else if (ws.band) {
        BandArgs ba;
        ba.sa = p.sa; ba.sb = p.sb; ba.x = p.x; ba.edge = (unsigned long long *)ws.edge.p; ba.gflags = p.flags; ba.err = c->d_err;
        ba.ent = ws.ent; ba.edge_job = ws.edge_job; ba.W = g.w; ba.H = g.h; ba.K = K; ba.NB = ws.NB; ba.NW = ws.NG; ba.RP = ws.RP; ba.G = ws.G;
        ba.lead = band_ring(ws.F);
        if (sw_given(Switches::SOR_LEAD)) ba.lead = std::max(band_ch(ws.F) + 2, std::min(sw_int(Switches::SOR_LEAD, 0), band_ring(ws.F)));
        ba.NS = ws.NS; ba.NCH = ws.NCH; ba.nb = g.nb; ba.Wp = ws.Wp; ba.EP = ws.EP; ba.omega = omega; ba.active = g.active; ba.amask = g.amask;
        const dim3 bgrid(g.nb * ws.NB), bblock(ws.NG * 64);
        const size_t tvb = (ws.F + 1) * band_ch(ws.F) <= 64 ? (size_t)(ws.F + 1) * band_ch(ws.F) * 8 : 0;
        const size_t lds = (size_t)(ws.NG - 1) * band_ring(ws.F) * 64 * 8 + 256 + ws.NG * band_window(ws.F) + (size_t)ws.NG * ws.F * band_mc(ws.F) * 8 + ws.NG * tvb;
        if (ws.band == 43) {
            const size_t lds43 = (size_t)7 * 16 * 64 * 8 + 256 + 6 * (size_t)(2 * 3 * 67 * 32) + 2 * (size_t)(2 * 2 * 66 * 32) + (size_t)8 * 4 * 12 * 8 + (size_t)8 * 5 * 4 * 8;
            hipLaunchKernelGGL((k_sor_band_mixed<4, 6, 3, 2, 4, 12, 16>), bgrid, bblock, lds43, c->stream, ba);
        } else if (ws.F == 6) hipLaunchKernelGGL((k_sor_band<6, 5, band_ch(6), band_mc(6), 16>), bgrid, bblock, lds, c->stream, ba);
        else if (ws.F == 5) hipLaunchKernelGGL((k_sor_band<5, 6, band_ch(5), band_mc(5), 16>), bgrid, bblock, lds, c->stream, ba);
        else if (ws.F == 3) hipLaunchKernelGGL((k_sor_band<3, 10, band_ch(3), band_mc(3), 16>), bgrid, bblock, lds, c->stream, ba);
        else if (ws.F == 2) hipLaunchKernelGGL((k_sor_band<2, 16, band_ch(2), band_mc(2), 8>), bgrid, bblock, lds, c->stream, ba);
        else                hipLaunchKernelGGL((k_sor_band<1, 16, band_ch(1), band_mc(1), 16>), bgrid, bblock, lds, c->stream, ba);
    }
#endif
    else {
    const dim3 sgrid(g.nb * ws.ntasks), sblock(64);
    if (ws.F == 1 && ws.CHK == 16)      hipLaunchKernelGGL((k_sor_solve<1, 16>), sgrid, sblock, 0, c->stream, a);
    SFA_FULL(else if (ws.F == 1)                 hipLaunchKernelGGL((k_sor_solve<1, 8>), sgrid, sblock, 0, c->stream, a);)
    else if (ws.F == 2 && ws.CHK == 8)  hipLaunchKernelGGL((k_sor_solve<2, 8>), sgrid, sblock, 0, c->stream, a);
    SFA_FULL(else if (ws.F == 2)                 hipLaunchKernelGGL((k_sor_solve<2, 4>), sgrid, sblock, 0, c->stream, a);)
    SFA_FULL(else if (ws.F == 3)                 hipLaunchKernelGGL((k_sor_solve<3, 4>), sgrid, sblock, 0, c->stream, a);)
    else return set_error(c, SFA_ERR_ARG, "sor_launch_solve: no task kernel of %d sweeps per wave in chunks of %d in this build", ws.F, ws.CHK);
    }
    if (prof) {
        (void)hipEventRecord(c->ev[c->ev_used + 1], c->stream);
        c->ev_used += 2;
        c->sor_bytes += (44.0 * K + 12.0) * (double)g.w * g.h * g.nb;
    }
    if (du)
        hipLaunchKernelGGL(k_sor_finish, dim3((g.w + 63) / 64, (g.h + 3) / 4, g.nb), dim3(64, 4), 0, c->stream, du, dv, p.x, ws.ent, g.es, g.w, g.h, ws.RP,
                           ws.G, g.pitch, g.active, g.amask);
    SFA_HIP(c, hipGetLastError());
    return SFA_OK;
}

}
```

### slowflow_amd/csrc/sor_chain.hip

```cpp
#include <atomic>
#include "sfa_internal.h"
#include "sfa_device.h"
#include "sor_device.h"

#pragma clang fp contract(off)

namespace sfa {

struct ChainArgs {
    const float4 *sa, *sb;
    unsigned long long *x, *edge;
    unsigned *gflags;
    const int2 *order;
    unsigned *err;
    long ent, edge_job;
    unsigned long long edge_bytes, flag_bytes;
    int W, H, K, NB, NG, RP, G, nb, Wp, EP;
    int nch;
    int NI;
    float omega;
    WMask active; const unsigned long long *amask;
};

constexpr int kFlagStride = 32;
constexpr unsigned kAuxSc1 = 16;

__device__ __forceinline__ unsigned long long bload8_sc1(__amdgpu_buffer_rsrc_t r, unsigned voff, unsigned soff) {
    const v2u v = __builtin_amdgcn_raw_buffer_load_b64(r, voff, soff, kAuxSc1);
    return (unsigned long long)v.x | ((unsigned long long)v.y << 32);
}
__device__ __forceinline__ void bstore8_sc1(__amdgpu_buffer_rsrc_t r, unsigned voff, unsigned soff, unsigned long long v) {
    v2u t = {(unsigned)v, (unsigned)(v >> 32)};
    __builtin_amdgcn_raw_buffer_store_b64(t, r, voff, soff, kAuxSc1);
}
__device__ __forceinline__ unsigned bload4_sc1(__amdgpu_buffer_rsrc_t r, unsigned voff, unsigned soff) { return __builtin_amdgcn_raw_buffer_load_b32(r, voff, soff, kAuxSc1); }
__device__ __forceinline__ void bstore4_sc1(__amdgpu_buffer_rsrc_t r, unsigned voff, unsigned soff, unsigned v) { __builtin_amdgcn_raw_buffer_store_b32(v, r, voff, soff, kAuxSc1); }

struct RsrcWords { v4u w; };
__device__ __forceinline__ RsrcWords rsrc_words(const void *base, unsigned long long bytes) {
    const unsigned long long p = (unsigned long long)base;
    RsrcWords r;
    r.w.x = __builtin_amdgcn_readfirstlane((unsigned)p);
    r.w.y = __builtin_amdgcn_readfirstlane((unsigned)(p >> 32)) & 0xffffu;
    r.w.z = __builtin_amdgcn_readfirstlane((unsigned)(bytes > 0xffffff00ull ? 0xffffff00ull : bytes));
    r.w.w = 0x00020000u;
    return r;
}
__device__ __forceinline__ void batomic_swap8(const RsrcWords &r, unsigned voff, unsigned soff, unsigned long long v) {
#ifdef SFA_X_OUT_NOATOM
    asm volatile("" ::"v"(v), "v"(voff), "s"(r.w), "s"(soff)); return;
#endif
    asm volatile("buffer_atomic_swap_x2 %0, %1, %2, %3 offen" ::"v"(v), "v"(voff), "s"(r.w), "s"(soff) : "memory");
}
__device__ __forceinline__ void batomic_umax4(const RsrcWords &r, unsigned voff, unsigned soff, unsigned v) {
// ... 14 lines not shown
    asm volatile("s_barrier" ::: "memory"); _t1 = __builtin_readcyclecounter(); acc += _t1 - _t0; accw += _t0 - _tw; } while (0)
#else
#define SFA_CHAIN_BARRIER_T(acc) SFA_CHAIN_BARRIER()
#define SFA_CHAIN_BARRIER_T2(acc, accw) SFA_CHAIN_BARRIER()
#endif

#ifndef SFA_CHAIN_OPRING
#define SFA_CHAIN_OPRING 1
#endif
__host__ __device__ constexpr int chain_start_shift(int KG) { return KG <= 10 ? 2 : 4; }
#ifndef SFA_CHAIN_PF
#define SFA_CHAIN_PF 2
#endif
#ifndef SFA_CHAIN_PFL
#define SFA_CHAIN_PFL 3
#endif
#ifndef SFA_CHAIN_PF1
#define SFA_CHAIN_PF1 4
#endif
template <int FA, int NA, int FB, int NB_>
struct ChainShape {
    static constexpr int NW = NA + NB_, KG = NA * FA + NB_ * FB, FMAX = FA > FB ? FA : FB;
    __host__ __device__ static constexpr int Fw(int w) { return w < NA ? FA : FB; }
    __host__ __device__ static constexpr int kw(int w) { return w < NA ? w * FA : NA * FA + (w - NA) * FB; }
    static constexpr bool MULTI = FA >= 2 && (NB_ == 0 || FB >= 2) && NW < 8, LONE = FA == 1 && NB_ == 0 && NW < 8;
#ifndef SFA_CHAIN_INFILL
#define SFA_CHAIN_INFILL 1
#endif
    static constexpr bool INFILL = SFA_CHAIN_INFILL && LONE && SFA_CHAIN_PF1 == 4;
    static constexpr int NWAVES = NW + 2 + (INFILL ? 1 : 0);
    static constexpr int PF0 = MULTI ? SFA_CHAIN_PF : LONE ? SFA_CHAIN_PF1 : 1;
    static constexpr int PFL = MULTI ? SFA_CHAIN_PFL : LONE ? SFA_CHAIN_PF1 : 1;
    static constexpr bool PERM9 = NW == 7 && NA == 1;
    static constexpr bool PERM9L = NW == 7 && NA == 6 && NB_ == 1;
#ifndef SFA_CHAIN_PERM6
#define SFA_CHAIN_PERM6 0
#endif
    __host__ __device__ static constexpr int stage_of_wave6(int wave) {
        return SFA_CHAIN_PERM6 == 1 ? (wave == 1 ? 2 : wave == 3 ? 0 : wave - 1) : SFA_CHAIN_PERM6 == 2 ? (wave == 4 ? 0 : wave == 1 ? 3 : wave - 1) : wave - 1;
    }
    static constexpr bool PERM12 = NW == 10 && NA == 5 && NB_ == 5 && FA == 2 && FB == 1;
    __host__ __device__ static constexpr int stage_of_wave12(int wave) {
        constexpr int m[11] = {-1, 0, 2, 4, 1, 5, 7, 9, 3, 6, 8};
        return m[wave];
    }
    __host__ __device__ static constexpr int stage_of_wave(int wave) {
        return PERM12 ? stage_of_wave12(wave) : PERM9 ? (wave == 4 ? 0 : wave < 4 ? wave : wave - 1) : PERM9L ? (wave == 4 ? 6 : wave < 4 ? wave - 1 : wave - 2) : NW == 6 ? stage_of_wave6(wave) : wave - 1;
    }
};

template <class S, int CH>
struct ChainLds {
    static constexpr int RING = 2 * CH * 64 * 8;
    static constexpr int ring0 = 0;
    static constexpr int tv0 = ring0 + (S::NW + 1) * RING;
    static constexpr int TVW = 2 * CH * (S::FMAX + 1) * 8;
    static constexpr int es0 = tv0 + S::NW * TVW;
    static constexpr int ESW = 2 * (S::FMAX > 1 ? S::FMAX - 1 : 1) * CH * 8;
    static constexpr int dummy0 = es0 + S::NW * ESW;
    static constexpr int DUMMY = 64 * 8 + ESW;
    static constexpr int OPW = 64 + S::KG - 1, OPROWB = OPW * 16, OPRMIN = 3 * (S::NW - 1) + 2 * (S::KG - 1) + 9;
    static constexpr int ops0 = (dummy0 + DUMMY + 15) & ~15;
    static constexpr bool OPR10 = ops0 + 2 * (OPRMIN + 1) * OPROWB + 32 <= 160 * 1024, OPR00 = ops0 + 2 * OPRMIN * OPROWB + 32 <= 160 * 1024;
    static constexpr int OPRTIGHT = 3 * S::NW + 2 * S::KG + 2 - (S::PFL < CH ? S::PFL - 1 : 0);
#ifndef SFA_X_OPR_CUT
#define SFA_X_OPR_CUT 0
// ... 6 lines not shown
    static_assert(!OPRING || !S::INFILL || (OPR % 4 == 0 && OPR >= OPRMIN + 1 + 8), "FILL wave: groups of four rows never wrap, and a group is in flight for two intervals");
    static constexpr int ticket = ops0 + (OPRING ? 2 * OPPLANE : 0);
    static constexpr int total = ticket + 16;
};

__device__ __forceinline__ v2f pk_mul_hi(v2f hi2, v2f b) {
    v2f r;
    asm("v_pk_mul_f32 %0, %1, %2 op_sel:[1,0] op_sel_hi:[1,1]" : "=v"(r) : "v"(hi2), "v"(b));
    return r;
}
template <bool SCALAR_T2 = true>
__device__ __forceinline__ v2f sor_point2(v2f self, v2f right, v2f top, v2f bottom, v2f left, v2f hlz, const float4 &SA, const float4 &SB, float omega) {
    const v2f SAxy = {SA.x, SA.y}, SAzw = {SA.z, SA.w}, SBxy = {SB.x, SB.y}, SBzw = {SB.z, SB.w};
#ifdef SFA_X_NOARITH
    return self + right * SAxy + top * SBxy + bottom * SAzw + left * hlz;
#endif
    v2f s = __builtin_shufflevector(SBzw, SBzw, 0, 0) * right;
    s = s + pk_mul_hi(SAzw, top);
    s = s + pk_mul_hi(SBzw, bottom);
    s = s + SBxy;
    const v2f B = __builtin_shufflevector(hlz, hlz, 0, 0) * left + s;
    v2f t2;
    if (SCALAR_T2) {
        float t2x, t2y;
        asm("v_mul_f32 %0, %1, %2" : "=v"(t2x) : "v"(SA.y), "v"(B.y));
        asm("v_mul_f32 %0, %1, %2" : "=v"(t2y) : "v"(SA.z), "v"(B.y));
        t2 = (v2f){t2x, t2y};
    } else
        t2 = (v2f){SA.y * B.y, SA.z * B.y};
    const v2f t = SAxy * __builtin_shufflevector(B, B, 0, 0) + t2;
    return self + omega * (t - self);
}

template <int F, int CH, int PD, bool SHORT = false, int ROLE = 0, int OPS0 = 0, int OPR = 1, int OPROWB = 0, int KG = 1, int PF_ = 1>
__device__ __forceinline__ void chain_compute(const ChainArgs &a, unsigned char *lds, int ring_in, int ring_out, int tvb, int esb, int dummy, int job, int b,
                                              int k0, int s_start, int lead, int lane, int kap0 = 0, int w = 0) {
    constexpr int OPPLANE = OPR * OPROWB;
    constexpr int F0 = ROLE == 2 ? 0 : 1;
    static_assert(PD % 2 == 0, "the chunk parity must be a compile-time constant of the body position");
    constexpr int P0 = (F >= 4 || SHORT) ? CH : PD * CH, P1 = (F <= 2 && !SHORT) ? P0 : CH;
    const int RP = a.RP;
    const float omega = a.omega;
    const int r0 = 64 * b - k0;
    const long FOFF = 2L * RP + 1;
    const long E0 = (long)(r0 + a.G) * RP + (r0 + a.G) + (long)s_start * RP - (long)(F - 1) * FOFF;
#ifdef SFA_X_NOLOAD
    const __amdgpu_buffer_rsrc_t rA = plane_rsrc(a.sa + (size_t)job * a.ent + E0, 0);
    const __amdgpu_buffer_rsrc_t rB = plane_rsrc(a.sb + (size_t)job * a.ent + E0, 0);
#else
    const __amdgpu_buffer_rsrc_t rA = plane_rsrc(a.sa + (size_t)job * a.ent + E0, 0xffffff00ull);
    const __amdgpu_buffer_rsrc_t rB = plane_rsrc(a.sb + (size_t)job * a.ent + E0, 0xffffff00ull);
#endif
    unsigned vo[F];
#pragma unroll
    for (int f = 0; f < F; f++) vo[f] = (unsigned)((lane + (F - 1 - f) * FOFF) * 16);
    const unsigned st16 = (unsigned)RP * 16u;
    unsigned so = 0;

    float4 sa0[ROLE == 2 ? 1 : P0], sb0[ROLE == 2 ? 1 : P0], sa1[(F > 1 && ROLE == 0) ? F - 1 : 1][ROLE == 0 ? P1 : 1], sb1[(F > 1 && ROLE == 0) ? F - 1 : 1][ROLE == 0 ? P1 : 1];
    if (ROLE != 2) {
#pragma unroll
        for (int j = 0; j < P0; j++) { sa0[j] = bload16(rA, vo[0], j * st16); sb0[j] = bload16(rB, vo[0], j * st16); }
    }
    if (ROLE == 0) {
#pragma unroll
        for (int f = 1; f < F; f++)
#pragma unroll
// ... 18 lines not shown
        for (int q = 0; q < NSL; q++) la[f][q] = lb[f][q] = make_float4(0.f, 0.f, 0.f, 0.f);
        if (ROLE != 0 && f >= F0) {
#pragma unroll
            for (int q = 0; q < PRE; q++) {
                la[f][q] = *reinterpret_cast<const float4 *>(lds + rd_lane[f] + rd_off[f]);
                lb[f][q] = *reinterpret_cast<const float4 *>(lds + rd_lane[f] + rd_off[f] + OPPLANE);
                rd_off[f] = rd_off[f] + OPROWB == (unsigned)OPPLANE ? 0u : rd_off[f] + OPROWB;
            }
        }
    }
    const unsigned wr_lane = (unsigned)(OPS0 + (KG - 1 + lane) * 16);
    float2 res[F], selfv[F];
    v2f hlz[F];
#pragma unroll
    for (int f = 0; f < F; f++) { res[f] = make_float2(0.f, 0.f); selfv[f] = make_float2(0.f, 0.f); hlz[f] = (v2f){0.f, 0.f}; }

    const unsigned long long *rin = reinterpret_cast<const unsigned long long *>(lds + ring_in) + lane;
    unsigned long long *rout = reinterpret_cast<unsigned long long *>(lds + ring_out) + lane;
    const unsigned long long *tvp = reinterpret_cast<const unsigned long long *>(lds + tvb);
    unsigned long long *esp = reinterpret_cast<unsigned long long *>(lds + (lane == 63 ? esb : dummy + lane * 8));

    int I = 0;
#ifdef SFA_CHAIN_TIMING
    unsigned long long t_begin = __builtin_readcyclecounter(), t_lead = 0, t_bar = 0, t_first = 0, t_last = 0, t_ldsrd = 0, t_wr = 0;
#endif
#ifndef SFA_CHAIN_CPRIO
#define SFA_CHAIN_CPRIO 0
#endif
    if (SFA_CHAIN_CPRIO) __builtin_amdgcn_s_setprio(SFA_CHAIN_CPRIO);
    for (; I < lead; I++) SFA_CHAIN_BARRIER_T(t_lead);
#ifdef SFA_CHAIN_TIMING
    t_first = __builtin_readcyclecounter();
#endif
    const int nbody = a.nch / PD;
    for (int body = 0; body < nbody; body++) {
#pragma unroll
        for (int q = 0; q < PD; q++) {
            SFA_CHAIN_BARRIER_T2(t_bar, t_wr);
            const int par = q & 1;
            constexpr bool JIT = F >= 4;
            unsigned long long bot[CH], fl[CH][F + 1];
            if (!JIT) {
#pragma unroll
                for (int j = 0; j < CH; j++) {
                    bot[j] = rin[(par * CH + j) * 64];
#pragma unroll
                    for (int fi = 0; fi <= F; fi++) fl[j][fi] = tvp[(par * CH + j) * (F + 1) + fi];
                }
            }
            if (CHUNK_AHEAD) {
#pragma unroll
                for (int f = 0; f < F; f++)
#pragma unroll
                    for (int j = 1; j <= CH; j++) {
                        la[f][(q * CH + j) % NSL] = *reinterpret_cast<const float4 *>(lds + rd_lane[f] + rd_off[f]);
                        lb[f][(q * CH + j) % NSL] = *reinterpret_cast<const float4 *>(lds + rd_lane[f] + rd_off[f] + OPPLANE);
                        rd_off[f] = rd_off[f] + OPROWB == (unsigned)OPPLANE ? 0u : rd_off[f] + OPROWB;
                    }
            }
#ifdef SFA_CHAIN_TIMING
            {
                unsigned long long ta = __builtin_readcyclecounter();
                asm volatile("s_waitcnt lgkmcnt(0)" ::: "memory");
                t_ldsrd += __builtin_readcyclecounter() - ta;
            }
#endif
#pragma unroll
            for (int j = 0; j < CH; j++) {
                const int j0 = (q * CH + j) % P0, j1 = (q * CH + j) % P1;
                const int p0 = (j0 + P0 - 1) % P0, p1 = (j1 + P1 - 1) % P1;
                if (JIT) {
                    bot[j] = rin[(par * CH + j) * 64];
#pragma unroll
                    for (int fi = 0; fi <= F; fi++) fl[j][fi] = tvp[(par * CH + j) * (F + 1) + fi];
                    asm volatile("" ::: "memory");
                }
                const float2 bottom0 = u2f(bot[j]);
                float2 sh[F], right0;
                { const float2 t = u2f(fl[j][0]); right0.x = lane_shr1(bottom0.x, t.x); right0.y = lane_shr1(bottom0.y, t.y); }
#pragma unroll
                for (int f = 0; f < F; f++) { const float2 t = u2f(fl[j][f + 1]); sh[f].x = lane_shr1(res[f].x, t.x); sh[f].y = lane_shr1(res[f].y, t.y); }
                float2 nres[F];
#pragma unroll
                for (int f = 0; f < F; f++) {
                    const float2 right = f == 0 ? right0 : sh[f > 0 ? f - 1 : 0];
                    const float2 bottom = f == 0 ? bottom0 : res[f > 0 ? f - 1 : 0];
                    const bool ringfed = ROLE != 0 && f >= F0;
                    const float4 &SA = ringfed ? la[f][(CHUNK_AHEAD ? q * CH + j : j) % NSL] : f == 0 ? sa0[ROLE == 2 ? 0 : j0] : sa1[(f > 0 && ROLE == 0) ? f - 1 : 0][ROLE == 0 ? j1 : 0];
                    const float4 &SB = ringfed ? lb[f][(CHUNK_AHEAD ? q * CH + j : j) % NSL] : f == 0 ? sb0[ROLE == 2 ? 0 : j0] : sb1[(f > 0 && ROLE == 0) ? f - 1 : 0][ROLE == 0 ? j1 : 0];
                    const v2f xn = sor_point2<(F >= 2)>(f2v(selfv[f]), f2v(right), f2v(sh[f]), f2v(bottom), f2v(res[f]), hlz[f], SA, SB, omega);
                    nres[f] = make_float2(xn.x, xn.y);
                    selfv[f] = right;
                }
#pragma unroll
                for (int f = 0; f < F; f++) res[f] = nres[f];
#pragma unroll
                for (int f = 0; f + 1 < F; f++) esp[(par * (F - 1) + f) * CH + j] = f2u(res[f].x, res[f].y);
                rout[(par * CH + j) * 64] = f2u(res[F - 1].x, res[F - 1].y);
#ifdef SFA_X_NORINGWR
                if (false) {
#else
                if (ROLE == 1) {
#endif
                    *reinterpret_cast<float4 *>(lds + wr_lane + wr_off) = sa0[j0];
                    *reinterpret_cast<float4 *>(lds + wr_lane + wr_off + OPPLANE) = sb0[j0];
                    wr_off = wr_off + OPROWB == (unsigned)OPPLANE ? 0u : wr_off + OPROWB;
                }
                if (ROLE != 2) { sa0[p0] = bload16(rA, vo[0], so + (P0 - 1) * st16); sb0[p0] = bload16(rB, vo[0], so + (P0 - 1) * st16); }
                if (ROLE == 0) {
#pragma unroll
                    for (int f = 1; f < F; f++) { sa1[f - 1][p1] = bload16(rA, vo[f], so + (P1 - 1) * st16); sb1[f - 1][p1] = bload16(rB, vo[f], so + (P1 - 1) * st16); }
                }
#pragma unroll
                for (int f = 0; f < F; f++) {
                    const bool ringfed = ROLE != 0 && f >= F0;
                    if (ringfed) {
                        hlz[f] = (v2f){lb[f][(CHUNK_AHEAD ? q * CH + j : j) % NSL].z, lb[f][(CHUNK_AHEAD ? q * CH + j : j) % NSL].w};
#ifdef SFA_X_NORINGRD
                        if (false) {
#else
                        if (!CHUNK_AHEAD) {
#endif
                            la[f][(j + PF) % NSL] = *reinterpret_cast<const float4 *>(lds + rd_lane[f] + rd_off[f]);
                            lb[f][(j + PF) % NSL] = *reinterpret_cast<const float4 *>(lds + rd_lane[f] + rd_off[f] + OPPLANE);
#ifndef SFA_X_NOWRAP
                            rd_off[f] = rd_off[f] + OPROWB == (unsigned)OPPLANE ? 0u : rd_off[f] + OPROWB;
#endif
                        }
                    } else if (f == 0) hlz[0] = (v2f){sb0[ROLE == 2 ? 0 : j0].z, sb0[ROLE == 2 ? 0 : j0].w};
                    else hlz[f] = (v2f){sb1[(f > 0 && ROLE == 0) ? f - 1 : 0][ROLE == 0 ? j1 : 0].z, sb1[(f > 0 && ROLE == 0) ? f - 1 : 0][ROLE == 0 ? j1 : 0].w};
                }
                so += st16;
            }
        }
    }
    I += a.nch;
#ifdef SFA_CHAIN_TIMING
    t_last = __builtin_readcyclecounter();
    if (job == 0 && lane == 0 && (int)blockIdx.x < 64) {
        unsigned long long *o = g_chain_timing + ((size_t)blockIdx.x * 16 + (threadIdx.x >> 6)) * 16;
        o[0] = t_begin; o[1] = t_first; o[2] = t_last; o[3] = t_lead; o[4] = t_bar; o[5] = (unsigned long long)b; o[6] = (unsigned long long)k0; o[7] = (unsigned long long)a.nch;
        o[8] = t_ldsrd; o[9] = t_wr; o[13] = __builtin_amdgcn_s_getreg((31 << 11) | 4); o[14] = __builtin_amdgcn_s_getreg((31 << 11) | 20);
    }
#endif
    for (; I < a.NI; I++) SFA_CHAIN_BARRIER();
}

__device__ __forceinline__ unsigned chain_wait(__amdgpu_buffer_rsrc_t rF, unsigned voff, unsigned soff, unsigned target, unsigned *err, bool &dead) {
    unsigned spins = 0, limit = kSpinLimit;
    for (;;) {
        const unsigned v = __builtin_amdgcn_readfirstlane(bload4_sc1(rF, voff, soff));
        if (v >= target || dead) return v;
        if (spins == 0) {
            const unsigned o = ld_flag(err + 1);
            if (o) limit = o;
        }
        __builtin_amdgcn_s_sleep(1);
        if ((++spins & 1023u) == 0 || spins > limit) {
            const unsigned e = ld_flag(err);
            if (e || spins > limit) {
                if ((threadIdx.x & 63) == 0) __hip_atomic_store(err, 1u, __ATOMIC_RELAXED, __HIP_MEMORY_SCOPE_AGENT);
                dead = true;
                return v;
            }
        }
    }
// ... 182 lines not shown
    constexpr int NQ = CH * L::OPW, ND = (NQ + 63) / 64;
    static_assert(2 * ND <= 63, "vmcnt is a 6-bit counter");
    const ChainGeo<S, CH> G(a, b, g, c_first);
    const long e0 = (long)job * a.ent + G.U00 + (long)G.s_start0 * G.RP - (S::KG - 1);
    const unsigned lds0 = (unsigned)(size_t)(const __attribute__((address_space(3))) void *)(lds + L::ops0);
    unsigned voff[ND];
    bool on[ND];
#pragma unroll
    for (int k = 0; k < ND; k++) {
        const int n = 64 * k + lane, j = n / L::OPW, e = n % L::OPW;
        on[k] = n < NQ;
        voff[k] = (unsigned)((j * G.RP + e) * 16);
    }
    const float4 *pa = a.sa + e0, *pb = a.sb + e0;
    const long step = (long)CH * G.RP;
    int row = 0;
    for (int I = 0; I < a.NI; I++) {
        SFA_CHAIN_BARRIER();
        const unsigned dst = lds0 + (unsigned)row * (unsigned)L::OPROWB;
#pragma unroll
        for (int k = 0; k < ND; k++) {
            if (on[k]) {
                chain_dma16(pa, voff[k], dst + 1024u * k);
                chain_dma16(pb, voff[k], dst + (unsigned)L::OPPLANE + 1024u * k);
            }
        }
        asm volatile("s_waitcnt vmcnt(%0)" ::"n"(2 * ND) : "memory");
        pa += step; pb += step;
        row = row + CH >= L::OPR ? 0 : row + CH;
    }
    asm volatile("s_waitcnt vmcnt(0)" ::: "memory");
}

template <class S, int CH, int AH, int PUBD>
__device__ __forceinline__ void chain_out(const ChainArgs &a, unsigned char *lds, int job, int b, int g, int c_first, int lane) {
    using L = ChainLds<S, CH>;
    constexpr int NW = S::NW, LEAD = AH + 1, Fl = S::Fw(NW - 1);
    constexpr int NES = [] { int n = 0; for (int w = 0; w < NW; w++) n += S::Fw(w) * CH; return n; }();
    constexpr int NSE = (NES + 63) / 64;
    constexpr int T = NSE + CH + 1;
    static_assert(PUBD * T <= 63, "vmcnt is a 6-bit counter");
    const ChainGeo<S, CH> G(a, b, g, c_first);
    const int RP = G.RP, K = G.K, W = G.W, H = G.H;
    const RsrcWords rE = rsrc_words(a.edge, a.edge_bytes);
    const RsrcWords rF = rsrc_words(a.gflags, a.flag_bytes);
    const RsrcWords rXout = rsrc_words(a.x + (size_t)job * a.ent + G.U0l + (long)G.s_startl * RP - (long)(Fl - 1) * G.FOFF, 0xffffff00ull);
    unsigned es_voff[NSE], es_lds[NSE][2];
    int es_lo[NSE];
#pragma unroll
    for (int n = 0; n < NSE; n++) {
        const int i = n * 64 + lane;
        int w = 0, base = 0;
        while (w < NW - 1 && i >= base + S::Fw(w) * CH) { base += S::Fw(w) * CH; w++; }
        const int Fw = S::Fw(w), rel = i - base, f = rel / CH, j = rel % CH;
        const bool on = i < NES;
        const int k0w = G.k0g + S::kw(w), Ow = k0w - (G.st0 + w) + 1;
        const int s0 = (c_first - 1 - LEAD - w) * CH - Ow;
        const long off = (long)job * a.edge_job + ((long)b * K + k0w + f) * a.Wp + a.EP + (s0 + j - 63 - f);
        es_voff[n] = on ? (unsigned)(off * 8) : kOobOffset;
        es_lo[n] = on ? LEAD + w + 1 : 0x7fffffff;
#pragma unroll
        for (int p = 0; p < 2; p++) {
            const int cp = (p + w) & 1;
            es_lds[n][p] = !on ? (unsigned)(L::dummy0 + lane * 8)
                         : f < Fw - 1 ? (unsigned)(L::es0 + w * L::ESW + ((cp * (Fw - 1) + f) * CH + j) * 8)
                                      : (unsigned)(L::ring0 + (w + 1) * L::RING + ((cp * CH + j) * 64 + 63) * 8);
        }
    }
    const int rl = G.r0l + lane - (Fl - 1);
#ifdef SFA_X_NOXSTORE
    const unsigned vXout = kOobOffset; (void)rl;
#else
    const unsigned vXout = (rl >= 0 && rl < H) ? (unsigned)lane * 8u : kOobOffset;
#endif
    const int lanef = lane + (Fl - 1);
    const unsigned st8 = (unsigned)RP * 8u;
    const unsigned vF0 = lane == 0 ? 0u : kOobOffset;
    const unsigned so_mine = (unsigned)((((size_t)job * a.NB + b) * a.NG + g) * 4 * kFlagStride);
    unsigned so_es = 0, so_xout = 0;
    int s_out = G.s_startl - (LEAD + NW) * CH;
    unsigned char *const ldsb = lds;
#ifdef SFA_CHAIN_TIMING
    unsigned long long t_begin = __builtin_readcyclecounter(), t_bar = 0, t_pub = 0, t0, t1;
#endif
    for (int I0 = 0; I0 < a.NI; I0 += 2) {
#pragma unroll
        for (int q = 0; q < 2; q++) {
            const int I = I0 + q;
            const int p = q & 1;
            SFA_CHAIN_BARRIER_T(t_bar);
#pragma unroll
            for (int n = 0; n < NSE; n++) {
#ifdef SFA_X_OUT_NOLDS
                const unsigned long long v = (unsigned long long)I + es_lds[n][p];
#else
                const unsigned long long v = *reinterpret_cast<const unsigned long long *>(ldsb + es_lds[n][p]);
#endif
                const bool act = I >= es_lo[n] && I < es_lo[n] + a.nch;
                batomic_swap8(rE, act ? es_voff[n] : kOobOffset, so_es, v);
            }
            {
                const bool act = I >= LEAD + NW && I < LEAD + NW + a.nch;
                const int po = (p + NW - 1) & 1;
                const unsigned long long *rp = reinterpret_cast<const unsigned long long *>(ldsb + L::ring0 + NW * L::RING + (po * CH * 64) * 8) + lane;
#pragma unroll
                for (int j = 0; j < CH; j++) {
                    const bool ok = act && (unsigned)(s_out + j - lanef) < (unsigned)W;
                    batomic_swap8(rXout, ok ? vXout : kOobOffset, so_xout + (unsigned)j * st8, rp[j * 64]);
                }
            }
#ifdef SFA_CHAIN_TIMING
            SFA_CT_STAMP(t0);
#endif
            asm volatile("s_waitcnt vmcnt(%0)" ::"n"(PUBD * T - 1) : "memory");
#ifdef SFA_CHAIN_TIMING
            SFA_CT_STAMP(t1); t_pub += t1 - t0;
#endif
            batomic_umax4(rF, vF0, so_mine, (unsigned)max(I - PUBD + 1, 0));
            so_es += CH * 8u; s_out += CH;
            if (I >= LEAD + NW) so_xout += CH * st8;
        }
    }
#ifdef SFA_CHAIN_TIMING
    if (job == 0 && lane == 0 && (int)blockIdx.x < 64) {
        unsigned long long *o = g_chain_timing + ((size_t)blockIdx.x * 16 + (threadIdx.x >> 6)) * 16;
        o[0] = t_begin; o[1] = __builtin_readcyclecounter(); o[2] = t_bar; o[4] = t_pub;
        o[9] = (unsigned long long)b; o[10] = (unsigned long long)g; o[11] = (unsigned long long)a.NI; o[12] = 0x20ull;
        o[13] = __builtin_amdgcn_s_getreg((31 << 11) | 4); o[14] = __builtin_amdgcn_s_getreg((31 << 11) | 20);
    }
#endif
    asm volatile("s_waitcnt vmcnt(0)" ::: "memory");
    batomic_umax4(rF, vF0, so_mine, 0x7fffffffu);
}

template <int FA, int NA, int FB, int NB_, int CH, int PD, int AH, int PL, int PUBD>
#ifdef SFA_CHAIN_WAVES_PER_EU
__attribute__((amdgpu_waves_per_eu(SFA_CHAIN_WAVES_PER_EU, SFA_CHAIN_WAVES_PER_EU)))
#endif
__global__ void __launch_bounds__((ChainShape<FA, NA, FB, NB_>::NWAVES * 64)) k_sor_chain(ChainArgs a) {
    using S = ChainShape<FA, NA, FB, NB_>;
    using L = ChainLds<S, CH>;
    constexpr int NW = S::NW, LEAD = AH + 1;
    extern __shared__ __attribute__((aligned(16))) unsigned char smem[];
    const int lane = threadIdx.x & 63;
    const int wave = __builtin_amdgcn_readfirstlane(threadIdx.x >> 6);
    unsigned *s_ticket = reinterpret_cast<unsigned *>(smem + L::ticket);
    if (threadIdx.x == 0) *s_ticket = atomicAdd(a.gflags + (size_t)a.nb * a.NB * a.NG * kFlagStride, 1u);
    for (int i = threadIdx.x; i < L::ticket / 8; i += S::NWAVES * 64) reinterpret_cast<unsigned long long *>(smem)[i] = 0ull;
    __syncthreads();
    const unsigned t = __builtin_amdgcn_readfirstlane(*s_ticket);
    if (t >= (unsigned)(a.nb * a.NB * a.NG)) return;
    const int job = t % a.nb;
    if (!elem_active(a.active, a.amask, job)) return;
    const int2 bg = a.order[t / a.nb];
    const int b = __builtin_amdgcn_readfirstlane(bg.x), g = __builtin_amdgcn_readfirstlane(bg.y);
    constexpr int SHIFT = L::OPRING ? chain_start_shift(S::KG) : 0;
    const int c_first = (((g * (S::KG - NW)) / CH) & ~1) - SHIFT;
    const int c_first_prev = g > 0 ? ((((g - 1) * (S::KG - NW)) / CH) & ~1) - SHIFT : 0;
#ifdef SFA_X_NOIO
#ifdef SFA_X_NOIO_POLL
    if (wave == 0) {
        const __amdgpu_buffer_rsrc_t rF = plane_rsrc(a.gflags, a.flag_bytes);
        const unsigned so = (unsigned)((((size_t)job * a.NB + b) * a.NG + g) * 4);
        unsigned acc = 0, pend[4] = {0, 0, 0, 0};
        for (int I = 0; I < a.NI; I += 4) {
#pragma unroll
            for (int q = 0; q < 4; q++) {
                SFA_CHAIN_BARRIER();
                acc += pend[(q + 1) % 4];
#if SFA_X_NOIO_POLL == 1
                pend[q] = bload4_sc1(rF, lane == 0 ? 0u : kOobOffset, so);
#elif SFA_X_NOIO_POLL == 2
                pend[q] = __builtin_amdgcn_raw_buffer_load_b32(rF, lane == 0 ? 0u : kOobOffset, so, 0);
#elif SFA_X_NOIO_POLL == 3
                bstore4_sc1(rF, lane == 0 ? 0u : kOobOffset, so, (unsigned)I);
#elif SFA_X_NOIO_POLL == 4
                __builtin_amdgcn_raw_buffer_store_b32((unsigned)I, rF, lane == 0 ? 0u : kOobOffset, so, 0);
#elif SFA_X_NOIO_POLL == 5
                __builtin_amdgcn_raw_buffer_store_b32((unsigned)I, rF, lane == 0 ? 0u : kOobOffset, so, 2);
#elif SFA_X_NOIO_POLL == 6
                __builtin_amdgcn_raw_buffer_store_b32((unsigned)I, rF, lane == 0 ? 0u : kOobOffset, so, 17);
#elif SFA_X_NOIO_POLL == 7
                if (lane == 0) __hip_atomic_fetch_add(a.gflags + so / 4, 1u, __ATOMIC_RELAXED, __HIP_MEMORY_SCOPE_AGENT);
#elif SFA_X_NOIO_POLL == 8
                { const __amdgpu_buffer_rsrc_t rX8 = plane_rsrc(a.x + (size_t)job * a.ent, 0xffffff00ull); bstore8_sc1(rX8, lane * 8u, (unsigned)(I & 7) * 512u, 0ull); }
#elif SFA_X_NOIO_POLL == 10
// ... 32 lines not shown
                    const __amdgpu_buffer_rsrc_t rX8 = plane_rsrc(a.x + (size_t)job * a.ent + (size_t)blockIdx.x * 4096, 0xffffff00ull);
                    unsigned long long r = 0;
#pragma unroll
                    for (int j = 0; j < 4; j++) r ^= bload8_sc1(rX8, lane * 8u, (unsigned)(j * 512 + (I & 15) * 2048));
                    pend[q] = (unsigned)r;
                }
#elif SFA_X_NOIO_POLL == 16
                {
                    unsigned long long *xp = a.x + (size_t)job * a.ent + (size_t)blockIdx.x * 4096 + lane;
#pragma unroll
                    for (int j = 0; j < 4; j++) __hip_atomic_exchange(xp + j * 64, (unsigned long long)I, __ATOMIC_RELAXED, __HIP_MEMORY_SCOPE_AGENT);
                    if (lane < 12) __hip_atomic_exchange(a.edge + (size_t)blockIdx.x * 64 + lane, (unsigned long long)I, __ATOMIC_RELAXED, __HIP_MEMORY_SCOPE_AGENT);
                    asm volatile("s_waitcnt vmcnt(14)" ::: "memory");
                    if (lane == 0) __hip_atomic_fetch_max(a.gflags + so / 4, (unsigned)I, __ATOMIC_RELAXED, __HIP_MEMORY_SCOPE_AGENT);
                }
#elif SFA_X_NOIO_POLL == 9
                { const __amdgpu_buffer_rsrc_t rX8 = plane_rsrc(a.x + (size_t)job * a.ent, 0xffffff00ull); v2u z = {0u, 0u}; __builtin_amdgcn_raw_buffer_store_b64(z, rX8, lane * 8u, (unsigned)(I & 7) * 512u, 0); }
#endif
            }
        }
        if (acc == 0x12345678u) bstore4_sc1(rF, 0u, so, acc);
        return;
    }
#endif
    if (wave == 0 || wave == NW + 1) { for (int I = 0; I < a.NI; I++) SFA_CHAIN_BARRIER(); return; }
#endif
#ifdef SFA_X_IN_IDLE
    if (wave == 0) { for (int I = 0; I < a.NI; I++) SFA_CHAIN_BARRIER(); return; }
#endif
#ifdef SFA_X_OUT_IDLE
    if (wave == NW + 1) { for (int I = 0; I < a.NI; I++) SFA_CHAIN_BARRIER(); return; }
#endif
    if (wave == 0) { chain_in<S, CH, AH, PL>(a, smem, job, b, g, c_first, c_first_prev, lane); return; }
    if (wave == NW + 1) { chain_out<S, CH, AH, PUBD>(a, smem, job, b, g, c_first, lane); return; }
    if (S::INFILL && wave == NW + 2) { if constexpr (S::INFILL) chain_fill<S, CH, AH>(a, smem, job, b, g, c_first, lane); return; }
    const int w = S::stage_of_wave(wave);
    const int st = g * NW + w, k0 = g * S::KG + S::kw(w), O = k0 - st + 1;
    const int s_start = c_first * CH - O;
    const int ring_in = L::ring0 + w * L::RING, ring_out = ring_in + L::RING;
    const int tvb = L::tv0 + w * L::TVW, esb = L::es0 + w * L::ESW;
    constexpr bool SHORT = NW >= 8;
    constexpr int PF0 = S::PF0, PFL = S::PFL;
    if (L::OPRING) {
        if (w == 0)      chain_compute<FA, CH, PD, SHORT, S::INFILL ? 2 : 1, L::ops0, L::OPR, L::OPROWB, S::KG, PF0>(a, smem, ring_in, ring_out, tvb, esb, L::dummy0, job, b, k0, s_start, LEAD + w, lane, 0, 0);
        else if (w < NA) chain_compute<FA, CH, PD, SHORT, 2, L::ops0, L::OPR, L::OPROWB, S::KG, PFL>(a, smem, ring_in, ring_out, tvb, esb, L::dummy0, job, b, k0, s_start, LEAD + w, lane, S::kw(w), w);
        else             chain_compute<FB, CH, PD, SHORT, 2, L::ops0, L::OPR, L::OPROWB, S::KG, PFL>(a, smem, ring_in, ring_out, tvb, esb, L::dummy0, job, b, k0, s_start, LEAD + w, lane, S::kw(w), w);
    } else if (w < NA) chain_compute<FA, CH, PD, SHORT>(a, smem, ring_in, ring_out, tvb, esb, L::dummy0, job, b, k0, s_start, LEAD + w, lane);
    else               chain_compute<FB, CH, PD, SHORT>(a, smem, ring_in, ring_out, tvb, esb, L::dummy0, job, b, k0, s_start, LEAD + w, lane);
}

#ifndef SFA_CHAIN_AH
#define SFA_CHAIN_AH 2
#endif
#ifndef SFA_CHAIN_PL
#define SFA_CHAIN_PL 2
#endif
#ifndef SFA_CHAIN_PUBD
#define SFA_CHAIN_PUBD 2
#endif
constexpr int kChainCH = 4, kChainAH = SFA_CHAIN_AH, kChainPL = SFA_CHAIN_PL, kChainPUBD = SFA_CHAIN_PUBD;

struct ChainShapeInfo { int id, FA, NA, FB, NB_, PD, PL, PUBD; };
static const ChainShapeInfo kChainShapes[] = {
    SFA_FULL({1, 1, 3, 1, 0, 4, 2, 2},)
    SFA_FULL({2, 2, 3, 2, 0, 2, 2, 2},)
    SFA_FULL({3, 3, 5, 3, 0, 2, 2, 2},)
    SFA_FULL({5, 2, 5, 2, 0, 2, 2, 2},)
    {6, 1, 5, 1, 0, 4, 2, 2},
    SFA_FULL({8, 3, 2, 3, 0, 2, 2, 2},)
    SFA_FULL({9, 5, 6, 5, 0, 2, 2, 2},)
    SFA_FULL({10, 3, 10, 3, 0, 2, 2, 2},)
    SFA_FULL({11, 3, 3, 2, 3, 2, 1, 1},)
    SFA_FULL({12, 2, 3, 3, 3, 2, 2, 2},)
    SFA_FULL({13, 3, 1, 2, 6, 2, 1, 1},)
    {16, 1, 5, 1, 0, 4, 1, 1},
    SFA_FULL({17, 1, 3, 1, 0, 4, 1, 1},)
// ... 22 lines not shown
                snprintf(buf, n, "k_sor_chain<%d,%d,%d,%d,%d,%d,%d,%d,%d> (%d stages of %d + %d of %d sweeps, %d groups per band)", s.FA, s.NA, s.FB, s.NB_, kChainCH, s.PD, kChainAH,
                         s.PL, s.PUBD, s.NA, s.FA, s.NB_, s.FB, NG);
            else
                snprintf(buf, n, "k_sor_chain<%d,%d,%d,%d,%d,%d,%d,%d,%d> (%d stages of %d sweeps, %d groups per band)", s.FA, s.NA, s.FB, s.NB_, kChainCH, s.PD, kChainAH, s.PL, s.PUBD,
                         s.NA + s.NB_, s.FA, NG);
            return;
        }
    snprintf(buf, n, "k_sor_chain shape %d", id);
}
template <int FA, int NA, int FB, int NB_> static int shape_shift() { using S = ChainShape<FA, NA, FB, NB_>; return ChainLds<S, kChainCH>::OPRING ? chain_start_shift(S::KG) : 0; }
int chain_shift(int id) {
    switch (id) {
        SFA_FULL(case 1: return shape_shift<1, 3, 1, 0>();)
        SFA_FULL(case 2: return shape_shift<2, 3, 2, 0>();)
        SFA_FULL(case 3: return shape_shift<3, 5, 3, 0>();)
        SFA_FULL(case 5: return shape_shift<2, 5, 2, 0>();)
        case 6: return shape_shift<1, 5, 1, 0>();
        SFA_FULL(case 8: return shape_shift<3, 2, 3, 0>();)
        SFA_FULL(case 9: return shape_shift<5, 6, 5, 0>();)
        SFA_FULL(case 10: return shape_shift<3, 10, 3, 0>();)
        SFA_FULL(case 11: return shape_shift<3, 3, 2, 3>();)
        case 16: return shape_shift<1, 5, 1, 0>();
        SFA_FULL(case 12: return shape_shift<2, 3, 3, 3>();)
        SFA_FULL(case 13: return shape_shift<3, 1, 2, 6>();)
        SFA_FULL(case 17: return shape_shift<1, 3, 1, 0>();)
        SFA_FULL(case 19: return shape_shift<1, 6, 1, 0>();)
        case 14: return shape_shift<2, 6, 3, 1>();
#ifdef SFA_WHATIF_SHAPE20
        case 20: static_assert(ChainLds<ChainShape<2, 5, 1, 5>, kChainCH>::OPRING, "the what-if needs -DSFA_X_OPR_CUT=18: its ring does not fit"); return shape_shift<2, 5, 1, 5>();
#endif
    }
    return 0;
}
int chain_flag_stride() { return kFlagStride; }
int chain_ah() { return kChainAH; }

template <int FA, int NA, int FB, int NB_, int PD, int PL = kChainPL, int PUBD = kChainPUBD>
static int chain_launch_shape(sfa_ctx *c, const ChainArgs &a, int nwg) {
    using S = ChainShape<FA, NA, FB, NB_>;
    using L = ChainLds<S, kChainCH>;
    size_t lds = L::total;
    lds = std::max(lds, (size_t)sw_int(Switches::CHAIN_LDS, 0));
    static std::atomic<unsigned long long> attr_set{0};
    const bool tracked = c->device >= 0 && c->device < 64;
    const unsigned long long bit = tracked ? 1ull << c->device : 0ull;
    if (lds > 64 * 1024 && !(attr_set.load(std::memory_order_relaxed) & bit)) {
        const hipError_t e = hipFuncSetAttribute(reinterpret_cast<const void *>(&k_sor_chain<FA, NA, FB, NB_, kChainCH, PD, kChainAH, PL, PUBD>),
                                                 hipFuncAttributeMaxDynamicSharedMemorySize, (int)lds);
        if (e != hipSuccess)
            return set_error(c, SFA_ERR_HIP, "k_sor_chain<%d,%d,%d,%d>: %zu bytes of LDS per workgroup refused on device %d: %s", FA, NA, FB, NB_, lds, c->device,
                             hipGetErrorString(e));
        attr_set.fetch_or(bit, std::memory_order_relaxed);
    }
    hipLaunchKernelGGL((k_sor_chain<FA, NA, FB, NB_, kChainCH, PD, kChainAH, PL, PUBD>), dim3(nwg), dim3(S::NWAVES * 64), lds, c->stream, a);
    return SFA_OK;
}

int sor_chain_launch(sfa_ctx *c, SorWorkspace &ws, const Geo &g, int K, float omega) {
    ChainArgs a;
    a.sa = (const float4 *)ws.sa.p; a.sb = (const float4 *)ws.sb.p; a.x = (unsigned long long *)ws.x.p; a.edge = (unsigned long long *)ws.edge.p;
    a.gflags = (unsigned *)ws.flags.p; a.order = (const int2 *)ws.order.p; a.err = c->d_err;
    a.ent = ws.ent; a.edge_job = ws.edge_job; a.edge_bytes = (unsigned long long)g.nb * ws.edge_job * 8ull;
    a.flag_bytes = ((unsigned long long)g.nb * ws.nwords + 16) * 4ull;
    a.W = g.w; a.H = g.h; a.K = K; a.NB = ws.NB; a.NG = ws.NG; a.RP = ws.RP; a.G = ws.G; a.nb = g.nb; a.Wp = ws.Wp; a.EP = ws.EP;
    a.nch = ws.NCH; a.NI = ws.NS; a.omega = omega; a.active = g.active; a.amask = g.amask;
    const int nwg = g.nb * ws.NB * ws.NG;
    switch (ws.chain) {
        SFA_FULL(case 1: return chain_launch_shape<1, 3, 1, 0, 4>(c, a, nwg);)
        SFA_FULL(case 2: return chain_launch_shape<2, 3, 2, 0, 2>(c, a, nwg);)
        SFA_FULL(case 3: return chain_launch_shape<3, 5, 3, 0, 2>(c, a, nwg);)
        SFA_FULL(case 5: return chain_launch_shape<2, 5, 2, 0, 2>(c, a, nwg);)
        case 6: return chain_launch_shape<1, 5, 1, 0, 4>(c, a, nwg);
        SFA_FULL(case 8: return chain_launch_shape<3, 2, 3, 0, 2>(c, a, nwg);)
        SFA_FULL(case 9: return chain_launch_shape<5, 6, 5, 0, 2>(c, a, nwg);)
        SFA_FULL(case 10: return chain_launch_shape<3, 10, 3, 0, 2>(c, a, nwg);)
        SFA_FULL(case 11: return chain_launch_shape<3, 3, 2, 3, 2, 1, 1>(c, a, nwg);)
        case 16: return chain_launch_shape<1, 5, 1, 0, 4, 1, 1>(c, a, nwg);
        SFA_FULL(case 12: return chain_launch_shape<2, 3, 3, 3, 2>(c, a, nwg);)
        SFA_FULL(case 13: return chain_launch_shape<3, 1, 2, 6, 2, 1, 1>(c, a, nwg);)
        SFA_FULL(case 17: return chain_launch_shape<1, 3, 1, 0, 4, 1, 1>(c, a, nwg);)
        SFA_FULL(case 19: return chain_launch_shape<1, 6, 1, 0, 4, 1, 1>(c, a, nwg);)
        case 14: return chain_launch_shape<2, 6, 3, 1, 2, 1, 1>(c, a, nwg);
#ifdef SFA_WHATIF_SHAPE20
        case 20: return chain_launch_shape<2, 5, 1, 5, 2, 1, 1>(c, a, nwg);
#endif
        default: return set_error(c, SFA_ERR_ARG, "sor_chain_launch: unknown shape %d", ws.chain);
    }
}

}

#ifdef SFA_CHAIN_TIMING
extern "C" int sfa_debug_chain_timing(unsigned long long *out) { return (int)hipMemcpyFromSymbol(out, HIP_SYMBOL(sfa::g_chain_timing), sizeof(unsigned long long) * 64 * 16 * 16); }
#endif
```

### slowflow_amd/csrc/sor_device.h

```cpp
#pragma once
#include "sfa_internal.h"
#include "sfa_device.h"

#pragma clang fp contract(off)

namespace sfa {

constexpr unsigned kSpinLimit = 1u << 22;

__device__ __forceinline__ float2 u2f(unsigned long long v) { return make_float2(__uint_as_float((unsigned)v), __uint_as_float((unsigned)(v >> 32))); }
__device__ __forceinline__ unsigned long long f2u(float a, float b) { return (unsigned long long)__float_as_uint(a) | ((unsigned long long)__float_as_uint(b) << 32); }

typedef float v2f __attribute__((ext_vector_type(2)));
__device__ __forceinline__ v2f f2v(float2 a) { return (v2f){a.x, a.y}; }
__device__ __forceinline__ v2f sor_point(v2f self, v2f right, v2f top, v2f bottom, v2f left, float hl, const float4 &SA, const float4 &SB, float omega) {
    const v2f SAxy = {SA.x, SA.y}, SAzw = {SA.z, SA.w}, SBxy = {SB.x, SB.y}, SBzw = {SB.z, SB.w};
#ifdef SFA_X_NOARITH
    return self + right * SAxy + top * SBxy + bottom * SAzw + left * hl;
#endif
    v2f s = __builtin_shufflevector(SBzw, SBzw, 0, 0) * right;
    s = s + __builtin_shufflevector(SAzw, SAzw, 1, 1) * top;
    s = s + __builtin_shufflevector(SBzw, SBzw, 1, 1) * bottom;
    s = s + SBxy;
    const v2f B = hl * left + s;
    const v2f t = SAxy * __builtin_shufflevector(B, B, 0, 0) + __builtin_shufflevector(SAxy, SAzw, 1, 2) * __builtin_shufflevector(B, B, 1, 1);
    return self + omega * (t - self);
}

struct PointBlock { float dpsis, i11, i12, i22; };
__device__ __forceinline__ PointBlock sor_point_block(float hl, float hp, float vt, float vp, int r, int h, float a11, float a12, float a22) {
    PointBlock p;
    p.dpsis = hl + hp;
    if (r > 0) p.dpsis = p.dpsis + vt;
    if (r < h - 1) p.dpsis = p.dpsis + vp;
    const float A11 = a22 + p.dpsis, A22 = a11 + p.dpsis;
    const float det = A11 * A22 - a12 * a12;
    p.i11 = __fdiv_rn(A11, det); p.i22 = __fdiv_rn(A22, det); p.i12 = __fdiv_rn(a12, -det);
    return p;
}
__device__ __forceinline__ size_t diag_entry(int b, long ent, int RP, int G, int c, int r) { return (size_t)b * ent + (size_t)(c + r + G) * RP + (r + G); }

__device__ __forceinline__ float lane_shr1(float v, float fill) {
    return __int_as_float(__builtin_amdgcn_update_dpp(__float_as_int(fill), __float_as_int(v), 0x138 , 0xf, 0xf, false));
}

template <int X>
__device__ __forceinline__ int row0_from(int v) {
    if constexpr (X == 0) return v;
    else return __builtin_amdgcn_mov_dpp(v, 0x100 + X , 0x1, 0xf, false);
}
__device__ __forceinline__ int lane0_from(int v, int X) {
    switch (X) {
        case 0: return row0_from<0>(v);   case 1: return row0_from<1>(v);   case 2: return row0_from<2>(v);   case 3: return row0_from<3>(v);
        case 4: return row0_from<4>(v);   case 5: return row0_from<5>(v);   case 6: return row0_from<6>(v);   case 7: return row0_from<7>(v);
        case 8: return row0_from<8>(v);   case 9: return row0_from<9>(v);   case 10: return row0_from<10>(v); case 11: return row0_from<11>(v);
        case 12: return row0_from<12>(v); case 13: return row0_from<13>(v); case 14: return row0_from<14>(v); default: return row0_from<15>(v);
    }
}
__device__ __forceinline__ float lane_shr1_vec(float v, int fillvec) {
    return __int_as_float(__builtin_amdgcn_update_dpp(fillvec, __float_as_int(v), 0x138 , 0xf, 0xf, false));
}

__device__ __forceinline__ unsigned long long ld_x(const unsigned long long *p) {
    return __hip_atomic_load(p, __ATOMIC_RELAXED, __HIP_MEMORY_SCOPE_AGENT);
}
__device__ __forceinline__ void st_x(unsigned long long *p, unsigned long long v) {
    __hip_atomic_store(p, v, __ATOMIC_RELAXED, __HIP_MEMORY_SCOPE_AGENT);
}
__device__ __forceinline__ unsigned ld_flag(const unsigned *p) {
    return __builtin_amdgcn_readfirstlane(__hip_atomic_load(p, __ATOMIC_RELAXED, __HIP_MEMORY_SCOPE_AGENT));
}

typedef unsigned v4u __attribute__((ext_vector_type(4)));
// ... 47 lines not shown
```

Baseline: 262,600.

## Pack several batch elements side by side into one wide SOR chain train

Adds a 'train' mode in which up to 8 batch elements are laid out horizontally with a small gap in a single diagonal workspace. One chain wavefront pipeline then sweeps all of them, and a per-element active mask guards output writes. A cost model picks the train size from band count, CU count and chain step count, so fewer, longer chains fill the device while pipeline fill and drain overhead is amortized. It adds layout indexing (tsh/tpitch) to every diag_entry access and a new templated compute path. It is disabled when passengers or an explicit chain switch are present.

```diff
diff --git a/include/slowflow_amd.h b/include/slowflow_amd.h
--- a/include/slowflow_amd.h
+++ b/include/slowflow_amd.h
@@ -319,12 +319,14 @@
 int  sfa_sor_batch_upload(sfa_sor_batch *sb, int b, const float *du, const float *dv, const float *a11, const float *a12,
                           const float *a22, const float *b1, const float *b2, const float *sh, const float *sv, int stride);
 int  sfa_sor_batch_run(sfa_sor_batch *sb, int iterations, float omega);
+int  sfa_sor_batch_train(const sfa_sor_batch *sb);
 int  sfa_sor_batch_download(sfa_sor_batch *sb, int b, float *du, float *dv, int stride);
 
 int  sfa_ctx_set_wait_bound(sfa_ctx *ctx, unsigned spins);
 
 int  sfa_debug_set(const char *name, const char *value);
 int  sfa_ctx_set_verbose(sfa_ctx *ctx, int on);
+int  sfa_debug_sor_geometry(int w, int h, int K, int nb, int chain, int n, long long *out);
 
 int  sfa_pair_job_download_system(sfa_pair_job *job, int b, float *a11, float *a12, float *a22, float *b1, float *b2, int stride);
 
diff --git a/slowflow_amd/__init__.py b/slowflow_amd/__init__.py
--- a/slowflow_amd/__init__.py
+++ b/slowflow_amd/__init__.py
@@ -178,10 +178,10 @@
     "sfa_job_create", "sfa_job_destroy", "sfa_job_upload", "sfa_job_upload_resident", "sfa_job_reset_flow", "sfa_job_run", "sfa_job_download", "sfa_job_download_occlusions", "sfa_job_keep_alternation_occlusions", "sfa_job_download_alternation_occlusions", "sfa_job_mpix_iters", "sfa_job_device_bytes",
     "sfa_dev_layout_default", "sfa_job_upload_device", "sfa_job_set_flow_device", "sfa_job_download_device", "sfa_job_changes", "sfa_pair_job_upload_device", "sfa_pair_job_set_flow_device", "sfa_pair_job_download_device", "sfa_sequence_upload_device", "sfa_ctx_wait_stream", "sfa_ctx_signal_stream",
     "sfa_demosaic_device", "sfa_sequence_upload_mosaic_device", "sfa_sequence_upload_mosaic", "sfa_job_set_raw_weights", "sfa_sequence_rescale",
-    "sfa_sor_batch_create", "sfa_sor_batch_destroy", "sfa_sor_batch_upload", "sfa_sor_batch_run", "sfa_sor_batch_download",
+    "sfa_sor_batch_create", "sfa_sor_batch_destroy", "sfa_sor_batch_upload", "sfa_sor_batch_run", "sfa_sor_batch_train", "sfa_sor_batch_download",
     "sfa_track_params_default", "sfa_track_job_bytes", "sfa_track_job_create", "sfa_track_job_destroy", "sfa_track_job_upload_flows", "sfa_track_job_upload_frames", "sfa_track_job_upload_flows_device", "sfa_track_job_upload_frames_device", "sfa_track_job_run", "sfa_track_job_download_rate", "sfa_track_job_download_fused", "sfa_track_job_download_best", "sfa_ctx_free_bytes", "sfa_track_job_download_device", "sfa_track_job_stage_ms", "sfa_track_job_upload_occlusions_device", "sfa_track_job_download_rate_device", "sfa_track_job_download_best_device",
     "sfa_track_fill_params_default", "sfa_track_job_bytes_fill", "sfa_track_job_create_fill", "sfa_track_job_upload_fill", "sfa_track_job_upload_fill_device", "sfa_track_job_download_fill", "sfa_track_job_fill_ms", "sfa_track_job_fill_info",
-    "sfa_division_chain", "sfa_ctx_set_wait_bound", "sfa_debug_set", "sfa_ctx_set_verbose", "sfa_profile_enable", "sfa_profile_read", "sfa_profile_read_kernels", "sfa_timer_start", "sfa_timer_stop",
+    "sfa_division_chain", "sfa_ctx_set_wait_bound", "sfa_debug_set", "sfa_debug_sor_geometry", "sfa_ctx_set_verbose", "sfa_profile_enable", "sfa_profile_read", "sfa_profile_read_kernels", "sfa_timer_start", "sfa_timer_stop",
 ]
 
 _lib = None
@@ -1284,6 +1284,9 @@
     def run(self, iterations, omega):
         self.ctx._ck(lib().sfa_sor_batch_run(self.h_, int(iterations), C.c_float(omega)), "sfa_sor_batch_run")
 
+    def train(self):
+        return int(lib().sfa_sor_batch_train(self.h_))
+
     def download(self, b):
         stride = stride_of(self.w)
         du, dv = np.zeros((self.h, stride), np.float32), np.zeros((self.h, stride), np.float32)
diff --git a/slowflow_amd/csrc/api.hip b/slowflow_amd/csrc/api.hip
--- a/slowflow_amd/csrc/api.hip
+++ b/slowflow_amd/csrc/api.hip
@@ -18,7 +18,8 @@
     "SFA_SOR_CHAIN", "SFA_SOR_BAND", "SFA_SOR_F", "SFA_SOR_CH", "SFA_SOR_LEAD", "SFA_CHAIN_LDS", "SFA_RB_TILE", "SFA_WARP_ALLJ", "SFA_NO_WARP_SMOOTH",
     "SFA_ASSEMBLE_GENERIC", "SFA_EXACT_DIV", "SFA_ASM_XCD", "SFA_NO_DIRECT_OPERANDS", "SFA_NO_UV_ALIAS", "SFA_DEBUG_ACTIVE", "SFA_UNFUSED", "SFA_SHARE_SOR",
     "SFA_PYRAMID_UNFUSED", "SFA_CUT_DISCHARGE", "SFA_CUT_INNER", "SFA_CUT_SUPER", "SFA_CUT_TAIL_INNER", "SFA_CUT_PER", "SFA_CUT_TAIL_PER", "SFA_CUT_TAIL_SUPER",
-    "SFA_CUT_DEBUG", "SFA_CUT_NO_TAIL", "SFA_CUT_TAIL", "SFA_NO_EXACT_BREAK", "SFA_PAIR_UNFUSED", "SFA_EPIC_FIT_PLAIN", "SFA_EPIC_NN_SET", "SFA_EPIC_NN_SLICE"};
+    "SFA_CUT_DEBUG", "SFA_CUT_NO_TAIL", "SFA_CUT_TAIL", "SFA_NO_EXACT_BREAK", "SFA_PAIR_UNFUSED", "SFA_EPIC_FIT_PLAIN", "SFA_EPIC_NN_SET", "SFA_EPIC_NN_SLICE",
+    "SFA_SOR_TRAIN"};
 static int set_switch(const char *name, const char *value) {
     for (int i = 0; i < Switches::N; i++)
         if (!strcmp(name, kSwitchNames[i])) {
@@ -612,6 +613,7 @@
     SFA_HIP(ctx, hipStreamSynchronize(ctx->stream));
     return SFA_OK;
 }
+int sfa_sor_batch_train(const sfa_sor_batch *sb) { return sb && sb->ws.ctx && sb->ws.chain ? sb->ws.train : 0; }
 int sfa_sor_batch_run(sfa_sor_batch *sb, int iterations, float omega) {
     sfa_ctx *ctx = sb ? sb->ctx : nullptr;
     CHECK_ARGS(sb, "null batch");
diff --git a/slowflow_amd/csrc/job.hip b/slowflow_amd/csrc/job.hip
--- a/slowflow_amd/csrc/job.hip
+++ b/slowflow_amd/csrc/job.hip
@@ -245,6 +245,7 @@
     bool need_toref[2 * SFA_MAX_REF] = {false};
     SFA_TRY(data_terms(c, L, p, cw, aa, need_toref));
     const LevelPlan P(c, L, p);
+    sorws.passengers = P.thres_out || P.thres_in;
     const OuterBreak brk{c, P.thres_out};
     const WMask all = WMask::first(L.nb);
     Geo g = L.geo(all);
diff --git a/slowflow_amd/csrc/kernels.hip b/slowflow_amd/csrc/kernels.hip
--- a/slowflow_amd/csrc/kernels.hip
+++ b/slowflow_amd/csrc/kernels.hip
@@ -1360,7 +1360,7 @@
         if (cl < 0 || cl >= DT_X) continue;
         const int r = r0 + rl, c = c0 + cl;
         if (r >= g.h || c >= g.w) continue;
-        const size_t e = diag_entry(b, op.ent, op.RP, op.G, c, r);
+        const size_t e = diag_entry(b, op.ent, op.RP, op.G, c, r, op.tsh, op.tpitch);
         if (SFA_X_AI & 64) continue;
         const float2 xv = T.X[rl][cl];
         op.sa[e] = T.A[rl][cl];
@@ -1592,7 +1592,7 @@
     }
 }
 __global__ void __launch_bounds__(BX *BY) k_update_inner_x(float *__restrict__ uu, float *__restrict__ vv, const float *__restrict__ wx, const float *__restrict__ wy,
-                                                            const unsigned long long *__restrict__ xs, long ent, int RP, int G, const float *__restrict__ odu,
+                                                            const unsigned long long *__restrict__ xs, long ent, int RP, int G, int tsh, long tpitch, const float *__restrict__ odu,
                                                             const float *__restrict__ odv, float *__restrict__ du_out, float *__restrict__ dv_out,
                                                             double *__restrict__ partial, float *__restrict__ dfa, float *__restrict__ dfb, Geo g) {
     const int b = blockIdx.z;
@@ -1601,7 +1601,7 @@
     if (elem_active(g, b) && x < g.w)
         for (int y = blockIdx.y * BY + threadIdx.y; y < g.h; y += gridDim.y * BY) {
             const size_t o = b * g.es + (size_t)y * g.pitch + x;
-            const unsigned long long xv = xs[diag_entry(b, ent, RP, G, x, y)];
+            const unsigned long long xv = xs[diag_entry(b, ent, RP, G, x, y, tsh, tpitch)];
             const float d = __uint_as_float((unsigned)(xv & 0xffffffffu)), e = __uint_as_float((unsigned)(xv >> 32));
             const float od = odu ? odu[o] : 0.0f, oe = odv ? odv[o] : 0.0f;
             sa += (double)fabsf(od - d);
@@ -1619,7 +1619,7 @@
 }
 template <bool FUSE>
 __global__ void __launch_bounds__(BX *BY) k_update_outer_x(float *__restrict__ uu, float *__restrict__ vv, float *__restrict__ wx, float *__restrict__ wy,
-                                                            const unsigned long long *__restrict__ xs, long ent, int RP, int G, double *__restrict__ partial,
+                                                            const unsigned long long *__restrict__ xs, long ent, int RP, int G, int tsh, long tpitch, double *__restrict__ partial,
                                                             double *__restrict__ out, unsigned *__restrict__ done, float *__restrict__ dfa, float *__restrict__ dfb, Geo g) {
     __shared__ unsigned long long tX[16][67];
     const int b = blockIdx.z;
@@ -1634,7 +1634,7 @@
                 const int dl = item / 16, rl = item % 16, cl = dl - rl;
                 if (cl < 0 || cl >= 64) continue;
                 const int r = r0 + rl, c = c0 + cl;
-                if (r < g.h && c < g.w) tX[rl][cl] = xs[diag_entry(b, ent, RP, G, c, r)];
+                if (r < g.h && c < g.w) tX[rl][cl] = xs[diag_entry(b, ent, RP, G, c, r, tsh, tpitch)];
             }
             __syncthreads();
             const int x = c0 + threadIdx.x;
@@ -1824,7 +1824,7 @@
                            const float *old_dv, float *du_out, float *dv_out, double *red, float *dfa, float *dfb) {
     dim3 grid = red_grid(g, g.nb);
     const int per_elem = grid.x * grid.y;
-    hipLaunchKernelGGL(k_update_inner_x, grid, block2d(), 0, c->stream, uu, vv, wx, wy, x.x, x.ent, x.RP, x.G, old_du, old_dv, du_out, dv_out, partials_of(c), dfa, dfb, g);
+    hipLaunchKernelGGL(k_update_inner_x, grid, block2d(), 0, c->stream, uu, vv, wx, wy, x.x, x.ent, x.RP, x.G, x.tsh, x.tpitch, old_du, old_dv, du_out, dv_out, partials_of(c), dfa, dfb, g);
     hipLaunchKernelGGL(k_reduce_partials, dim3(g.nb), dim3(256), 0, c->stream, partials_of(c), per_elem, red, g.active, g.amask);
 }
 constexpr int kFuseReduceWindows = 4;
@@ -1833,10 +1833,10 @@
     const int per_elem = grid.x * grid.y;
     unsigned *done = c->d_last->done;
     if (g.nb <= kFuseReduceWindows) {
-        hipLaunchKernelGGL(k_update_outer_x<true>, grid, block2d(), 0, c->stream, uu, vv, wx, wy, x.x, x.ent, x.RP, x.G, partials_of(c), red, done, dfa, dfb, g);
+        hipLaunchKernelGGL(k_update_outer_x<true>, grid, block2d(), 0, c->stream, uu, vv, wx, wy, x.x, x.ent, x.RP, x.G, x.tsh, x.tpitch, partials_of(c), red, done, dfa, dfb, g);
         return;
     }
-    hipLaunchKernelGGL(k_update_outer_x<false>, grid, block2d(), 0, c->stream, uu, vv, wx, wy, x.x, x.ent, x.RP, x.G, partials_of(c), red, done, dfa, dfb, g);
+    hipLaunchKernelGGL(k_update_outer_x<false>, grid, block2d(), 0, c->stream, uu, vv, wx, wy, x.x, x.ent, x.RP, x.G, x.tsh, x.tpitch, partials_of(c), red, done, dfa, dfb, g);
     hipLaunchKernelGGL(k_reduce_partials, dim3(g.nb), dim3(256), 0, c->stream, partials_of(c), per_elem, red, g.active, g.amask);
 }
 void launch_update_outer(sfa_ctx *c, const Geo &g, float *wx, float *wy, const float *uu, const float *vv, double *red, float *dfa, float *dfb) {
diff --git a/slowflow_amd/csrc/sfa_internal.h b/slowflow_amd/csrc/sfa_internal.h
--- a/slowflow_amd/csrc/sfa_internal.h
+++ b/slowflow_amd/csrc/sfa_internal.h
@@ -99,7 +99,7 @@
     enum Id {
         SOR_CHAIN, SOR_BAND, SOR_F, SOR_CH, SOR_LEAD, CHAIN_LDS, RB_TILE, WARP_ALLJ, NO_WARP_SMOOTH, ASSEMBLE_GENERIC, EXACT_DIV, ASM_XCD, NO_DIRECT_OPERANDS,
         NO_UV_ALIAS, DEBUG_ACTIVE, UNFUSED, SHARE_SOR, PYRAMID_UNFUSED, CUT_DISCHARGE, CUT_INNER, CUT_SUPER, CUT_TAIL_INNER, CUT_PER, CUT_TAIL_PER, CUT_TAIL_SUPER,
-        CUT_DEBUG, CUT_NO_TAIL, CUT_TAIL, NO_EXACT_BREAK, PAIR_UNFUSED, EPIC_FIT_PLAIN, EPIC_NN_SET, EPIC_NN_SLICE, N
+        CUT_DEBUG, CUT_NO_TAIL, CUT_TAIL, NO_EXACT_BREAK, PAIR_UNFUSED, EPIC_FIT_PLAIN, EPIC_NN_SET, EPIC_NN_SLICE, SOR_TRAIN, N
     };
     bool given[N] = {};
     int value[N] = {};
@@ -259,6 +259,7 @@
 struct SorOperandOut {
     float4 *sa = nullptr, *sb = nullptr; unsigned long long *x = nullptr; unsigned *flags = nullptr;
     long ent = 0; int RP = 0, G = 0, ntasks = 0, nb = 0;
+    int tsh = 0; long tpitch = 0;
 };
 struct Term {
     long stack_off; long mask_off; float hd, hg, s; int is_ref;
@@ -350,6 +351,8 @@
     int band = 0, Wp = 0, EP = 0;
     int chain = 0;
     long edge_job = 0;
+    int train = 1, tsh = 0, P = 0;
+    bool passengers = false;
     DevMem sa, sb, x, flags, order, edge;
     int configure(sfa_ctx *ctx, int w, int h, int K, int nb);
 };
diff --git a/slowflow_amd/csrc/sor.hip b/slowflow_amd/csrc/sor.hip
--- a/slowflow_amd/csrc/sor.hip
+++ b/slowflow_amd/csrc/sor.hip
@@ -550,6 +550,7 @@
     float *a11, *a12, *a22;
     long ent, es;
     int W, H, RP, ND, G, pitch, ntasks, nb, inv_out;
+    int tsh; long tpitch;
     WMask active; const unsigned long long *amask;
 };
 constexpr int PT_C = 64, PT_R = 16;
@@ -587,7 +588,7 @@
         if (cl < 0 || cl >= PT_C) continue;
         const int r = r0 + rl, c = c0 + cl;
         if (r >= p.H || c >= p.W) continue;
-        const size_t e = diag_entry(job, p.ent, p.RP, p.G, c, r);
+        const size_t e = diag_entry(job, p.ent, p.RP, p.G, c, r, p.tsh, p.tpitch);
         p.sa[e] = tA[rl][cl];
         p.sb[e] = tB[rl][cl];
         const float2 xv = tX[rl][cl];
@@ -596,11 +597,11 @@
 }
 
 __global__ void k_sor_finish(float *__restrict__ du, float *__restrict__ dv, const unsigned long long *__restrict__ x, long ent, long es, int W, int H,
-                             int RP, int G, int pitch, WMask active, const unsigned long long *__restrict__ amask) {
+                             int RP, int G, int pitch, int tsh, long tpitch, WMask active, const unsigned long long *__restrict__ amask) {
     const int job = blockIdx.z;
     const int c = blockIdx.x * 64 + threadIdx.x, r = blockIdx.y * 4 + threadIdx.y;
     if (c >= W || r >= H || !elem_active(active, amask, job)) return;
-    const float2 v = u2f(x[diag_entry(job, ent, RP, G, c, r)]);
+    const float2 v = u2f(x[diag_entry(job, ent, RP, G, c, r, tsh, tpitch)]);
     const size_t o = (size_t)job * es + (size_t)r * pitch + c;
     du[o] = v.x;
     dv[o] = v.y;
@@ -791,6 +792,7 @@
 bool chain_shape(int id, int K, int *KG, int *NW, int *FMAX);
 int chain_ch();
 int chain_shift(int id);
+bool chain_trains(int id);
 void chain_kernel_name(int id, int NG, char *buf, size_t n);
 int chain_flag_stride();
 int chain_ah();
@@ -859,46 +861,92 @@
     if (K % F != 0) { F = 1; CHK = 16; }
 }
 
+constexpr int kTrainGap = 2, kTrainMinPitch = 24;
+int train_pitch(int w) { return std::max(w + kTrainGap, kTrainMinPitch); }
+int train_width(int w, int n) { return n == 1 ? w : (n - 1) * train_pitch(w) + w; }
+struct ChainGeom { int NB, NG, G, RP, NCH, NS, ND, EP, Wp, P; long ent, edge_job; };
+static ChainGeom chain_geometry(int chain, int K, int w, int h, int train) {
+    ChainGeom o;
+    int KG, NW, FMAX;
+    chain_shape(chain, K, &KG, &NW, &FMAX);
+    const int CH = chain_ch(), AH = chain_ah(), LEAD = AH + 1;
+    o.P = train_pitch(w);
+    o.NB = (h + K - 1 + 63) / 64;
+    o.NG = K / KG;
+#ifndef SFA_GUARD_ALIGN
+#define SFA_GUARD_ALIGN 8
+#endif
+    o.G = round_up(K + 64, SFA_GUARD_ALIGN);
+    o.RP = round_up(h + 2 * o.G, 16);
+    o.NCH = round_up((train_width(w, train) + 64 + KG - NW + 2 * CH + FMAX + CH - 1) / CH + chain_shift(chain), 4);
+    o.NS = round_up(o.NCH + LEAD + NW + 2, AH);
+    o.ND = o.NS * CH + 64 * o.NB + o.G + 32;
+    o.ent = (long)o.ND * o.RP;
+    o.EP = 256;
+    o.Wp = round_up(o.EP + o.NS * CH + 64 + 2 * K + 64, 8);
+    o.edge_job = (long)o.NB * K * o.Wp;
+    return o;
+}
+static bool train_fits(int chain, int K, int nb, int w, int h, int n) {
+    if (n < 1 || n > 8 || (n & (n - 1)) || nb % n) return false;
+    if (n == 1) return true;
+    if (!chain_trains(chain)) return false;
+    const ChainGeom g = chain_geometry(chain, K, w, h, n);
+    const long long trains = nb / n, lim = 0xffffff00ll;
+    return g.ent * 16 < lim && trains * g.edge_job * 8 < lim && (trains * g.NB * g.NG * chain_flag_stride() + 16) * 4 < lim;
+}
+static int train_rule(int chain, int K, int nb, int w, int h, int cu_count);
+static int train_choice(sfa_ctx *c, int chain, int K, int nb, int w, int h, bool passengers) {
+    if (!chain) return 1;
+    if (sw_given(Switches::SOR_TRAIN)) { const int n = sw_int(Switches::SOR_TRAIN, 1); return train_fits(chain, K, nb, w, h, n) ? n : 1; }
+    if (passengers || sw_given(Switches::SOR_CHAIN)) return 1;
+    return train_rule(chain, K, nb, w, h, c->cu_count);
+}
+static int train_rule(int chain, int K, int nb, int w, int h, int cu_count) {
+    const int NBands = (h + K - 1 + 63) / 64;
+    if (nb * NBands <= 72) return 1;
+    int KG, NW, FMAX;
+    chain_shape(chain, K, &KG, &NW, &FMAX);
+    const long cus = std::max(cu_count, 1), per_window = (long)NBands * (K / KG);
+    long best = (nb * per_window + cus - 1) / cus * chain_geometry(chain, K, w, h, 1).NS;
+    int n = 1;
+    for (int cand = 2; cand <= 8; cand *= 2) {
+        if (!train_fits(chain, K, nb, w, h, cand) || nb / cand * per_window < cus) continue;
+        const long cost = (nb / cand * per_window + cus - 1) / cus * chain_geometry(chain, K, w, h, cand).NS;
+        if (cost * 100 < best * 94) { best = cost; n = cand; }
+    }
+    return n;
+}
+
 int SorWorkspace::configure(sfa_ctx *c, int w_, int h_, int K_, int nb_) {
     int F_, CH_;
     const int chain_ = chain_choice(K_, nb_, (h_ + K_ - 1 + 63) / 64);
+    const int train_ = train_choice(c, chain_, K_, nb_, w_, h_, passengers);
     const int band_ = chain_ ? 0 : band_shape(K_, nb_);
     if (chain_) { F_ = 0; CH_ = chain_ch(); }
     else if (band_ == 43) { F_ = 4; CH_ = 12; }
     else if (band_) { F_ = band_; CH_ = band_mc(band_); }
     else sor_shape(K_, nb_ * ((h_ + K_ - 1 + 63) / 64) * K_, F_, CH_);
-    if (ctx == c && w == w_ && h == h_ && K == K_ && nb == nb_ && F == F_ && CHK == CH_ && band == band_ && chain == chain_) return SFA_OK;
+    if (ctx == c && w == w_ && h == h_ && K == K_ && nb == nb_ && F == F_ && CHK == CH_ && band == band_ && chain == chain_ && train == train_) return SFA_OK;
     ctx = c; w = w_; h = h_; K = K_; nb = nb_; F = F_; CHK = CH_; band = band_; chain = chain_;
+    train = train_; tsh = train == 8 ? 3 : train == 4 ? 2 : train == 2 ? 1 : 0; P = train_pitch(w);
     NB = (h + K - 1 + 63) / 64;
     if (chain) {
-        int KG, NW, FMAX;
-        chain_shape(chain, K, &KG, &NW, &FMAX);
-        const int CH = chain_ch(), AH = chain_ah(), LEAD = AH + 1;
-        NG = K / KG;
-#ifndef SFA_GUARD_ALIGN
-#define SFA_GUARD_ALIGN 8
-#endif
-        G = round_up(K + 64, SFA_GUARD_ALIGN);
-        RP = round_up(h + 2 * G, 16);
-        NCH = round_up((w + 64 + KG - NW + 2 * CH + FMAX + CH - 1) / CH + chain_shift(chain), 4);
-        NS = round_up(NCH + LEAD + NW + 2, AH);
-        ND = NS * CH + 64 * NB + G + 32;
+        const ChainGeom cg = chain_geometry(chain, K, w, h, train);
+        const int nt = nb / train;
+        NG = cg.NG; G = cg.G; RP = cg.RP; NCH = cg.NCH; NS = cg.NS; ND = cg.ND; ent = cg.ent; EP = cg.EP; Wp = cg.Wp; edge_job = cg.edge_job;
         ntasks = NB * NG;
         nwords = ntasks * chain_flag_stride();
-        ent = (long)ND * RP;
-        EP = 256;
-        Wp = round_up(EP + NS * CH + 64 + 2 * K + 64, 8);
-        edge_job = (long)NB * K * Wp;
-        SFA_TRY(edge.alloc(c, (size_t)nb * edge_job * sizeof(unsigned long long)));
-        SFA_HIP(c, hipMemsetAsync(edge.p, 0, (size_t)nb * edge_job * sizeof(unsigned long long), c->stream));
-        SFA_TRY(sa.alloc(c, (size_t)nb * ent * sizeof(float4)));
-        SFA_TRY(sb.alloc(c, (size_t)nb * ent * sizeof(float4)));
-        SFA_TRY(x.alloc(c, (size_t)nb * ent * sizeof(unsigned long long)));
-        SFA_TRY(flags.alloc(c, ((size_t)nb * nwords + 16) * sizeof(unsigned)));
+        SFA_TRY(edge.alloc(c, (size_t)nt * edge_job * sizeof(unsigned long long)));
+        SFA_HIP(c, hipMemsetAsync(edge.p, 0, (size_t)nt * edge_job * sizeof(unsigned long long), c->stream));
+        SFA_TRY(sa.alloc(c, (size_t)nt * ent * sizeof(float4)));
+        SFA_TRY(sb.alloc(c, (size_t)nt * ent * sizeof(float4)));
+        SFA_TRY(x.alloc(c, (size_t)nt * ent * sizeof(unsigned long long)));
+        SFA_TRY(flags.alloc(c, ((size_t)nt * nwords + 16) * sizeof(unsigned)));
         SFA_TRY(order.alloc(c, (size_t)NB * NG * sizeof(int2)));
-        SFA_HIP(c, hipMemsetAsync(sa.p, 0, (size_t)nb * ent * sizeof(float4), c->stream));
-        SFA_HIP(c, hipMemsetAsync(sb.p, 0, (size_t)nb * ent * sizeof(float4), c->stream));
-        SFA_HIP(c, hipMemsetAsync(x.p, 0, (size_t)nb * ent * sizeof(unsigned long long), c->stream));
+        SFA_HIP(c, hipMemsetAsync(sa.p, 0, (size_t)nt * ent * sizeof(float4), c->stream));
+        SFA_HIP(c, hipMemsetAsync(sb.p, 0, (size_t)nt * ent * sizeof(float4), c->stream));
+        SFA_HIP(c, hipMemsetAsync(x.p, 0, (size_t)nt * ent * sizeof(unsigned long long), c->stream));
         std::vector<int2> ord;
         ord.reserve(NB * NG);
         for (int key = 0; key <= 3 * (NB - 1) + (NG - 1); key++)
@@ -951,7 +999,8 @@
     if (g.w < 2 || g.h < 2 || K < 1) return set_error(c, SFA_ERR_ARG, "sor_operand_target: system too small for the pipelined solver");
     SFA_TRY(ws.configure(c, g.w, g.h, K, g.nb));
     out->sa = (float4 *)ws.sa.p; out->sb = (float4 *)ws.sb.p; out->x = (unsigned long long *)ws.x.p; out->flags = (unsigned *)ws.flags.p;
-    out->ent = ws.ent; out->RP = ws.RP; out->G = ws.G; out->ntasks = ws.nwords; out->nb = g.nb;
+    out->ent = ws.ent; out->RP = ws.RP; out->G = ws.G; out->ntasks = ws.nwords / ws.train; out->nb = g.nb;
+    out->tsh = ws.tsh; out->tpitch = (long)ws.P * ws.RP;
     return SFA_OK;
 }
 
@@ -969,7 +1018,7 @@
     p.sa = (float4 *)ws.sa.p; p.sb = (float4 *)ws.sb.p; p.x = (unsigned long long *)ws.x.p; p.flags = (unsigned *)ws.flags.p;
     p.du = du; p.dv = dv; p.b1 = b1; p.b2 = b2; p.sh = sh; p.sv = sv; p.a11 = a11; p.a12 = a12; p.a22 = a22;
     p.ent = ws.ent; p.es = g.es; p.W = g.w; p.H = g.h; p.RP = ws.RP; p.ND = ws.ND; p.G = ws.G; p.pitch = g.pitch;
-    p.ntasks = ws.nwords; p.nb = g.nb; p.inv_out = inv_out ? 1 : 0; p.active = g.active; p.amask = g.amask;
+    p.ntasks = ws.nwords / ws.train; p.nb = g.nb; p.tsh = ws.tsh; p.tpitch = (long)ws.P * ws.RP; p.inv_out = inv_out ? 1 : 0; p.active = g.active; p.amask = g.amask;
     hipLaunchKernelGGL(k_sor_prepare, dim3((g.w + PT_C - 1) / PT_C, (g.h + PT_R - 1) / PT_R, g.nb), dim3(256), 0, c->stream, p);
     return sor_launch_solve(c, ws, g, du, dv, K, omega);
 }
@@ -1031,9 +1080,19 @@
     }
     if (du)
         hipLaunchKernelGGL(k_sor_finish, dim3((g.w + 63) / 64, (g.h + 3) / 4, g.nb), dim3(64, 4), 0, c->stream, du, dv, p.x, ws.ent, g.es, g.w, g.h, ws.RP,
-                           ws.G, g.pitch, g.active, g.amask);
+                           ws.G, g.pitch, ws.tsh, (long)ws.P * ws.RP, g.active, g.amask);
     SFA_HIP(c, hipGetLastError());
     return SFA_OK;
 }
 
 }
+
+extern "C" int sfa_debug_sor_geometry(int w, int h, int K, int nb, int chain, int n, long long *out) {
+    int KG, NW, FMAX;
+    if (!out || w < 2 || h < 2 || K < 1 || nb < 1 || !sfa::chain_shape(chain, K, &KG, &NW, &FMAX)) return -1;
+    const int t = n == 0 ? sfa::train_rule(chain, K, nb, w, h, 256) : sfa::train_fits(chain, K, nb, w, h, n) ? n : 1;
+    const sfa::ChainGeom g = sfa::chain_geometry(chain, K, w, h, t);
+    const long long v[12] = {t, g.P, g.NB, g.NG, g.G, g.RP, g.NCH, g.NS, g.ND, g.ent, g.Wp, g.edge_job};
+    for (int i = 0; i < 12; i++) out[i] = v[i];
+    return 0;
+}
diff --git a/slowflow_amd/csrc/sor_chain.hip b/slowflow_amd/csrc/sor_chain.hip
--- a/slowflow_amd/csrc/sor_chain.hip
+++ b/slowflow_amd/csrc/sor_chain.hip
@@ -20,6 +20,7 @@
     int NI;
     float omega;
     WMask active; const unsigned long long *amask;
+    int tn, tP;
 };
 
 constexpr int kFlagStride = 32;
@@ -100,6 +101,7 @@
     static constexpr int PF0 = MULTI ? SFA_CHAIN_PF : LONE ? SFA_CHAIN_PF1 : 1;
     static constexpr int PFL = MULTI ? SFA_CHAIN_PFL : LONE ? SFA_CHAIN_PF1 : 1;
     static constexpr bool PERM9 = NW == 7 && NA == 1;
+    static constexpr bool TRAINS = !PERM9;
     static constexpr bool PERM9L = NW == 7 && NA == 6 && NB_ == 1;
 #ifndef SFA_CHAIN_PERM6
 #define SFA_CHAIN_PERM6 0
@@ -172,7 +174,13 @@
     return self + omega * (t - self);
 }
 
-template <int F, int CH, int PD, bool SHORT = false, int ROLE = 0, int OPS0 = 0, int OPR = 1, int OPROWB = 0, int KG = 1, int PF_ = 1>
+__device__ __forceinline__ float zero_where(float v, unsigned long long m) {
+    float o;
+    asm("v_cndmask_b32 %0, %1, 0, %2" : "=v"(o) : "v"(v), "s"(m));
+    return o;
+}
+
+template <int F, int CH, int PD, bool SHORT = false, int ROLE = 0, int OPS0 = 0, int OPR = 1, int OPROWB = 0, int KG = 1, int PF_ = 1, bool TRAIN = false>
 __device__ __forceinline__ void chain_compute(const ChainArgs &a, unsigned char *lds, int ring_in, int ring_out, int tvb, int esb, int dummy, int job, int b,
                                               int k0, int s_start, int lead, int lane, int kap0 = 0, int w = 0) {
     constexpr int OPPLANE = OPR * OPROWB;
@@ -257,11 +265,16 @@
 #ifdef SFA_CHAIN_TIMING
     t_first = __builtin_readcyclecounter();
 #endif
+    static_assert(!TRAIN || (F <= 5 && CH == 4 && PD <= 4), "the body test covers steps + 0 .. 3 and sweeps - 0 .. 4; the column test wraps once (P >= 24, sor.hip)");
+    constexpr int LIM = 72 + CH * (PD - 1);
+    const int P = TRAIN ? a.tP : 1;
+    unsigned long long pat = 0;
+    if (TRAIN) for (int l = 0; l < 64; l += P) pat |= 1ull << l;
+    pat = ((unsigned long long)__builtin_amdgcn_readfirstlane((unsigned)(pat >> 32)) << 32) | (unsigned)__builtin_amdgcn_readfirstlane((unsigned)pat);
+    int sb = TRAIN ? __builtin_amdgcn_readfirstlane(((s_start + 4 + CH * (PD - 1)) % P + P) % P) : 0;
     const int nbody = a.nch / PD;
-    for (int body = 0; body < nbody; body++) {
-#pragma unroll
-        for (int q = 0; q < PD; q++) {
-            SFA_CHAIN_BARRIER_T2(t_bar, t_wr);
+    auto chunk = [&](const int q, const bool MASKED) __attribute__((always_inline)) {
+        {
             const int par = q & 1;
             constexpr bool JIT = F >= 4;
             unsigned long long bot[CH], fl[CH][F + 1];
@@ -319,6 +332,17 @@
                 }
 #pragma unroll
                 for (int f = 0; f < F; f++) res[f] = nres[f];
+                if constexpr (TRAIN) {
+                    if (MASKED) {
+#pragma unroll
+                        for (int f = 0; f < F; f++) {
+                            int t = sb - CH * (PD - 1 - q) - 3 + j - f;
+                            t = t < 0 ? t + P : t >= P ? t - P : t;
+                            const unsigned long long hit = t < 64 ? pat << t : 0ull;
+                            res[f].x = zero_where(res[f].x, hit); res[f].y = zero_where(res[f].y, hit);
+                        }
+                    }
+                }
 #pragma unroll
                 for (int f = 0; f + 1 < F; f++) esp[(par * (F - 1) + f) * CH + j] = f2u(res[f].x, res[f].y);
                 rout[(par * CH + j) * 64] = f2u(res[F - 1].x, res[F - 1].y);
@@ -357,6 +381,26 @@
                 }
                 so += st16;
             }
+        }
+    };
+    for (int body = 0; body < nbody;) {
+        if constexpr (TRAIN) {
+            for (; body < nbody && sb < LIM; body++) {
+#pragma unroll
+                for (int q = 0; q < PD; q++) {
+                    SFA_CHAIN_BARRIER_T2(t_bar, t_wr);
+                    chunk(q, true);
+                }
+                sb = sb + PD * CH >= P ? sb + PD * CH - P : sb + PD * CH;
+            }
+        }
+        for (; body < nbody && (!TRAIN || sb >= LIM); body++) {
+#pragma unroll
+            for (int q = 0; q < PD; q++) {
+                SFA_CHAIN_BARRIER_T2(t_bar, t_wr);
+                chunk(q, false);
+            }
+            if constexpr (TRAIN) sb = sb + PD * CH >= P ? sb + PD * CH - P : sb + PD * CH;
         }
     }
     I += a.nch;
@@ -605,8 +649,8 @@
     asm volatile("s_waitcnt vmcnt(0)" ::: "memory");
 }
 
-template <class S, int CH, int AH, int PUBD>
-__device__ __forceinline__ void chain_out(const ChainArgs &a, unsigned char *lds, int job, int b, int g, int c_first, int lane) {
+template <class S, int CH, int AH, int PUBD, bool TRAIN>
+__device__ __forceinline__ void chain_out(const ChainArgs &a, unsigned char *lds, int job, int b, int g, int c_first, int lane, unsigned am) {
     using L = ChainLds<S, CH>;
     constexpr int NW = S::NW, LEAD = AH + 1, Fl = S::Fw(NW - 1);
     constexpr int NES = [] { int n = 0; for (int w = 0; w < NW; w++) n += S::Fw(w) * CH; return n; }();
@@ -651,7 +695,11 @@
     const unsigned vF0 = lane == 0 ? 0u : kOobOffset;
     const unsigned so_mine = (unsigned)((((size_t)job * a.NB + b) * a.NG + g) * 4 * kFlagStride);
     unsigned so_es = 0, so_xout = 0;
+    const int P = a.tP;
     int s_out = G.s_startl - (LEAD + NW) * CH;
+    const int col0 = s_out - lanef;
+    int kq = col0 >= 0 ? col0 / P : -((P - 1 - col0) / P);
+    int pc = col0 - kq * P;
     unsigned char *const ldsb = lds;
 #ifdef SFA_CHAIN_TIMING
     unsigned long long t_begin = __builtin_readcyclecounter(), t_bar = 0, t_pub = 0, t0, t1;
@@ -676,10 +724,13 @@
                 const bool act = I >= LEAD + NW && I < LEAD + NW + a.nch;
                 const int po = (p + NW - 1) & 1;
                 const unsigned long long *rp = reinterpret_cast<const unsigned long long *>(ldsb + L::ring0 + NW * L::RING + (po * CH * 64) * 8) + lane;
+                const unsigned w0 = ((unsigned)kq < 8u && ((am >> kq) & 1u)) ? (unsigned)W : 0u;
+                const unsigned w1 = ((unsigned)(kq + 1) < 8u && ((am >> (kq + 1)) & 1u)) ? (unsigned)W : 0u;
+                const unsigned vb = act ? vXout : kOobOffset;
 #pragma unroll
                 for (int j = 0; j < CH; j++) {
-                    const bool ok = act && (unsigned)(s_out + j - lanef) < (unsigned)W;
-                    batomic_swap8(rXout, ok ? vXout : kOobOffset, so_xout + (unsigned)j * st8, rp[j * 64]);
+                    const bool ok = TRAIN ? (unsigned)(pc + j) < w0 || (unsigned)(pc + j - P) < w1 : (unsigned)(s_out + j - lanef) < (unsigned)W;
+                    batomic_swap8(rXout, ok ? vb : kOobOffset, so_xout + (unsigned)j * st8, rp[j * 64]);
                 }
             }
 #ifdef SFA_CHAIN_TIMING
@@ -690,7 +741,8 @@
             SFA_CT_STAMP(t1); t_pub += t1 - t0;
 #endif
             batomic_umax4(rF, vF0, so_mine, (unsigned)max(I - PUBD + 1, 0));
-            so_es += CH * 8u; s_out += CH;
+            so_es += CH * 8u; s_out += CH; pc += CH;
+            if (pc >= P) { pc -= P; kq++; }
             if (I >= LEAD + NW) so_xout += CH * st8;
         }
     }
@@ -724,7 +776,11 @@
     const unsigned t = __builtin_amdgcn_readfirstlane(*s_ticket);
     if (t >= (unsigned)(a.nb * a.NB * a.NG)) return;
     const int job = t % a.nb;
-    if (!elem_active(a.active, a.amask, job)) return;
+    unsigned am = 0;
+    for (int k = 0; k < a.tn; k++)
+        if (elem_active(a.active, a.amask, job * a.tn + k)) am |= 1u << k;
+    am = __builtin_amdgcn_readfirstlane(am);
+    if (!am) return;
     const int2 bg = a.order[t / a.nb];
     const int b = __builtin_amdgcn_readfirstlane(bg.x), g = __builtin_amdgcn_readfirstlane(bg.y);
     constexpr int SHIFT = L::OPRING ? chain_start_shift(S::KG) : 0;
@@ -823,7 +879,11 @@
     if (wave == NW + 1) { for (int I = 0; I < a.NI; I++) SFA_CHAIN_BARRIER(); return; }
 #endif
     if (wave == 0) { chain_in<S, CH, AH, PL>(a, smem, job, b, g, c_first, c_first_prev, lane); return; }
-    if (wave == NW + 1) { chain_out<S, CH, AH, PUBD>(a, smem, job, b, g, c_first, lane); return; }
+    if (wave == NW + 1) {
+        if (a.tn > 1) chain_out<S, CH, AH, PUBD, true>(a, smem, job, b, g, c_first, lane, am);
+        else chain_out<S, CH, AH, PUBD, false>(a, smem, job, b, g, c_first, lane, am);
+        return;
+    }
     if (S::INFILL && wave == NW + 2) { if constexpr (S::INFILL) chain_fill<S, CH, AH>(a, smem, job, b, g, c_first, lane); return; }
     const int w = S::stage_of_wave(wave);
     const int st = g * NW + w, k0 = g * S::KG + S::kw(w), O = k0 - st + 1;
@@ -832,7 +892,11 @@
     const int tvb = L::tv0 + w * L::TVW, esb = L::es0 + w * L::ESW;
     constexpr bool SHORT = NW >= 8;
     constexpr int PF0 = S::PF0, PFL = S::PFL;
-    if (L::OPRING) {
+    if (L::OPRING && S::TRAINS && a.tn > 1) {
+        if (w == 0)      chain_compute<FA, CH, PD, SHORT, S::INFILL ? 2 : 1, L::ops0, L::OPR, L::OPROWB, S::KG, PF0, true>(a, smem, ring_in, ring_out, tvb, esb, L::dummy0, job, b, k0, s_start, LEAD + w, lane, 0, 0);
+        else if (w < NA) chain_compute<FA, CH, PD, SHORT, 2, L::ops0, L::OPR, L::OPROWB, S::KG, PFL, true>(a, smem, ring_in, ring_out, tvb, esb, L::dummy0, job, b, k0, s_start, LEAD + w, lane, S::kw(w), w);
+        else             chain_compute<FB, CH, PD, SHORT, 2, L::ops0, L::OPR, L::OPROWB, S::KG, PFL, true>(a, smem, ring_in, ring_out, tvb, esb, L::dummy0, job, b, k0, s_start, LEAD + w, lane, S::kw(w), w);
+    } else if (L::OPRING) {
         if (w == 0)      chain_compute<FA, CH, PD, SHORT, S::INFILL ? 2 : 1, L::ops0, L::OPR, L::OPROWB, S::KG, PF0>(a, smem, ring_in, ring_out, tvb, esb, L::dummy0, job, b, k0, s_start, LEAD + w, lane, 0, 0);
         else if (w < NA) chain_compute<FA, CH, PD, SHORT, 2, L::ops0, L::OPR, L::OPROWB, S::KG, PFL>(a, smem, ring_in, ring_out, tvb, esb, L::dummy0, job, b, k0, s_start, LEAD + w, lane, S::kw(w), w);
         else             chain_compute<FB, CH, PD, SHORT, 2, L::ops0, L::OPR, L::OPROWB, S::KG, PFL>(a, smem, ring_in, ring_out, tvb, esb, L::dummy0, job, b, k0, s_start, LEAD + w, lane, S::kw(w), w);
@@ -921,6 +985,24 @@
     }
     return 0;
 }
+template <int FA, int NA, int FB, int NB_> static bool shape_trains() { using S = ChainShape<FA, NA, FB, NB_>; return ChainLds<S, kChainCH>::OPRING && S::TRAINS; }
+bool chain_trains(int id) {
+    switch (id) {
+        SFA_FULL(case 1: return shape_trains<1, 3, 1, 0>();)
+        SFA_FULL(case 2: return shape_trains<2, 3, 2, 0>();)
+        SFA_FULL(case 3: return shape_trains<3, 5, 3, 0>();)
+        SFA_FULL(case 5: return shape_trains<2, 5, 2, 0>();)
+        case 6: return shape_trains<1, 5, 1, 0>();
+        SFA_FULL(case 8: return shape_trains<3, 2, 3, 0>();)
+        SFA_FULL(case 11: return shape_trains<3, 3, 2, 3>();)
+        case 16: return shape_trains<1, 5, 1, 0>();
+        SFA_FULL(case 12: return shape_trains<2, 3, 3, 3>();)
+        SFA_FULL(case 17: return shape_trains<1, 3, 1, 0>();)
+        SFA_FULL(case 19: return shape_trains<1, 6, 1, 0>();)
+        case 14: return shape_trains<2, 6, 3, 1>();
+    }
+    return false;
+}
 int chain_flag_stride() { return kFlagStride; }
 int chain_ah() { return kChainAH; }
 
@@ -949,11 +1031,13 @@
     ChainArgs a;
     a.sa = (const float4 *)ws.sa.p; a.sb = (const float4 *)ws.sb.p; a.x = (unsigned long long *)ws.x.p; a.edge = (unsigned long long *)ws.edge.p;
     a.gflags = (unsigned *)ws.flags.p; a.order = (const int2 *)ws.order.p; a.err = c->d_err;
-    a.ent = ws.ent; a.edge_job = ws.edge_job; a.edge_bytes = (unsigned long long)g.nb * ws.edge_job * 8ull;
-    a.flag_bytes = ((unsigned long long)g.nb * ws.nwords + 16) * 4ull;
-    a.W = g.w; a.H = g.h; a.K = K; a.NB = ws.NB; a.NG = ws.NG; a.RP = ws.RP; a.G = ws.G; a.nb = g.nb; a.Wp = ws.Wp; a.EP = ws.EP;
+    const int nt = g.nb / ws.train;
+    a.ent = ws.ent; a.edge_job = ws.edge_job; a.edge_bytes = (unsigned long long)nt * ws.edge_job * 8ull;
+    a.flag_bytes = ((unsigned long long)nt * ws.nwords + 16) * 4ull;
+    a.W = g.w; a.H = g.h; a.K = K; a.NB = ws.NB; a.NG = ws.NG; a.RP = ws.RP; a.G = ws.G; a.nb = nt; a.Wp = ws.Wp; a.EP = ws.EP;
     a.nch = ws.NCH; a.NI = ws.NS; a.omega = omega; a.active = g.active; a.amask = g.amask;
-    const int nwg = g.nb * ws.NB * ws.NG;
+    a.tn = ws.train; a.tP = ws.train > 1 ? ws.P : 1 << 30;
+    const int nwg = nt * ws.NB * ws.NG;
     switch (ws.chain) {
         SFA_FULL(case 1: return chain_launch_shape<1, 3, 1, 0, 4>(c, a, nwg);)
         SFA_FULL(case 2: return chain_launch_shape<2, 3, 2, 0, 2>(c, a, nwg);)
diff --git a/slowflow_amd/csrc/sor_device.h b/slowflow_amd/csrc/sor_device.h
--- a/slowflow_amd/csrc/sor_device.h
+++ b/slowflow_amd/csrc/sor_device.h
@@ -38,7 +38,9 @@
     p.i11 = __fdiv_rn(A11, det); p.i22 = __fdiv_rn(A22, det); p.i12 = __fdiv_rn(a12, -det);
     return p;
 }
-__device__ __forceinline__ size_t diag_entry(int b, long ent, int RP, int G, int c, int r) { return (size_t)b * ent + (size_t)(c + r + G) * RP + (r + G); }
+__device__ __forceinline__ size_t diag_entry(int b, long ent, int RP, int G, int c, int r, int tsh = 0, long tpitch = 0) {
+    return (size_t)(b >> tsh) * ent + (size_t)(b & ((1 << tsh) - 1)) * tpitch + (size_t)(c + r + G) * RP + (r + G);
+}
 
 __device__ __forceinline__ float lane_shr1(float v, float fill) {
     return __int_as_float(__builtin_amdgcn_update_dpp(__float_as_int(fill), __float_as_int(v), 0x138 , 0xf, 0xf, false));
```

After: 265,400, median of 6. +1.1%, better.
